# IvanBanny/para-ortho-pca-bo

Measured on AMD Instinct MI355X. Metric: BO iterations/sec (incl. GP refit + EI opt), BBOB f15 d=40, higher is better.
Workload: dtype f64; 1 GPU; configs[1]: PCA_BO on BBOB f15 d=40, budget=450, n_DoE=120, EI, var_threshold=0.95; one run per GPU (run list f15/d40/instances 0..N-1 partitioned by pcabo.sharding), timed steps spread evenly over the 330 BO iterations of the run; num_restarts=10, raw_samples=512, batch_limit=5, maxiter=200, parallelism=run-parallel x1

## Files before the change

include/pcabo.h:

```cpp
#ifndef PCABO_H
#define PCABO_H

#include <stddef.h>
#include <stdint.h>

#ifdef __cplusplus
extern "C" {
#endif

typedef struct pcabo_ctx pcabo_ctx;

typedef enum {
  PCABO_OK = 0,
  PCABO_ERR_ARG = -1,
  PCABO_ERR_NOT_PD = -2,
  PCABO_ERR_HIP = -3,
  PCABO_ERR_NAN = -4,
  PCABO_ERR_TIMEOUT = -5
} pcabo_status;

enum { PCABO_KERNEL_MATERN52 = 0, PCABO_KERNEL_RBF = 1 };
enum { PCABO_ACQ_LOG_EI = 0, PCABO_ACQ_PI = 1, PCABO_ACQ_UCB = 2 };
enum { PCABO_PTR_HOST = 0, PCABO_PTR_DEVICE = 1 };

int pcabo_abi_version(void);

int pcabo_device_count(void);

int pcabo_ctx_create(int device, int max_n, int max_d, int max_q, pcabo_ctx** out);
int pcabo_ctx_destroy(pcabo_ctx* ctx);
int pcabo_set_pointer_mode(pcabo_ctx* ctx, int mode);
int pcabo_last_error(pcabo_ctx* ctx, char* buf, int buflen);

enum { PCABO_OPT_RESIDENT = 0, PCABO_OPT_BESTF_F32 = 1, PCABO_OPT_GROUP_ACQ = 2,
       PCABO_OPT_DEVICE_LBFGSB = 3 ,
       PCABO_OPT_HIDDEN_TAIL = 5  };
int pcabo_set_option(pcabo_ctx* ctx, int option, int value);

int pcabo_wpca(pcabo_ctx* ctx, const double* X, const double* f, const int64_t* ranks, int n, int d,
               int maximize, double var_threshold, int n_components, const double* noise,
               double* data_mean, double* pca_mean, double* comps, double* evr, int* k, double* Z);

int pcabo_gp_condition(pcabo_ctx* ctx, const double* Z, const double* y, int n, int k,
                       const double* norm_bounds, double lengthscale, double noise, int kernel);

int pcabo_gp_condition_begin(pcabo_ctx* ctx, const double* Z, const double* y, int n, int k,
                             const double* norm_bounds, double lengthscale, double noise, int kernel);
int pcabo_gp_condition_end(pcabo_ctx* ctx);

int pcabo_gp_condition_end_eval(pcabo_ctx* ctx, const double* Xq, int q, double best_f, int maximize, int acq,
                                double* val);

int pcabo_gp_mll(pcabo_ctx* ctx, const double* Z , const double* y, int n, int k,
                 const double* norm_bounds, int kernel, const double* theta , double* loss, double* grad );
#define PCABO_FIT_TASK_NOT_PD (-2)
#define PCABO_FIT_TASK_DOMAIN (-3)
int pcabo_gp_fit(pcabo_ctx* ctx, const double* Z, const double* y, int n, int k, const double* norm_bounds, int kernel,
                 double* theta_inout , double* loss, int* info );
int pcabo_gp_mll_ard(pcabo_ctx* ctx, const double* Z, const double* y, int n, int k, const double* norm_bounds, int kernel,
                     const double* theta , double* loss, double* grad );
int pcabo_gp_fit_ard(pcabo_ctx* ctx, const double* Z, const double* y, int n, int k, const double* norm_bounds, int kernel,
                     double* theta_inout , double* loss, int* info );

int pcabo_wpca_gp_condition_begin(pcabo_ctx* ctx, const double* X, const double* f, const int64_t* ranks, int n,
                                  int d, int maximize, double var_threshold, int n_components, const double* noise,
                                  const double* y, double lengthscale, double gp_noise, int kernel,
                                  double* data_mean, double* pca_mean, double* comps, double* evr, int* k);

int pcabo_wpca_results(pcabo_ctx* ctx, double* data_mean, double* pca_mean, double* comps, double* evr, int* k);

int pcabo_acq_bounds(pcabo_ctx* ctx, double* bounds);

int pcabo_acq_eval(pcabo_ctx* ctx, const double* Xq, int q, double best_f, int maximize, int acq,
                   double* val, double* grad);
int pcabo_logei(pcabo_ctx* ctx, const double* Xq, int q, double best_f, int maximize,
                double* val, double* grad);

enum { PCABO_POST_OBS_NOISE = 1 };
int pcabo_gp_posterior(pcabo_ctx* ctx, const double* Xq, int q, int flags, double* mean, double* var, double* cov);

enum { PCABO_POST_CENTRED = 2 };
#define PCABO_POST_MAX_SAMPLES 1024
int pcabo_gp_posterior_sample(pcabo_ctx* ctx, const double* Xq, int q, int flags, const double* base, int S,
                              double* samples, double* mean , double* jitter_used );

int pcabo_gp_loo(pcabo_ctx* ctx, double* mean , double* var , double* z , double* lpd , double* lpd_sum );

enum { PCABO_EXTEND_BELIEVER = 1 };
int pcabo_gp_extend(pcabo_ctx* ctx, const double* Zp, const double* yp, int p, int flags);
int pcabo_gp_truncate(pcabo_ctx* ctx, int n0);
int pcabo_gp_extended(pcabo_ctx* ctx, int* n_base , int* n );

int pcabo_optimize_acqf(pcabo_ctx* ctx, const double* ics, int num_restarts, int batch_limit,
                        const double* bounds, int maxiter, double best_f, int maximize, int acq,
                        double* cand, double* vals, int* info, int* failed);

int pcabo_inverse_map(pcabo_ctx* ctx, const double* z, double* x);

int pcabo_get_gp_state(pcabo_ctx* ctx, double* K_chol , double* Rinv ,
                       double* alpha , double* y_mean_std , double* norm_bounds );
int pcabo_get_gram(pcabo_ctx* ctx, double* K );

typedef double (*pcabo_fg_callback)(const double* x, double* g, void* user);
int pcabo_lbfgsb_minimize(int nvar, double* x, const double* lower, const double* upper,
                          pcabo_fg_callback fg, void* user, int m, double factr, double pgtol,
                          int maxiter, int maxfun, int maxls, double* f_out, int* nit, int* nfev,
                          int* task_out);
int pcabo_lbfgsb_set_vector_kernels(int enabled);
int pcabo_lbfgsb_set_sum_order(int order);

int pcabo_sobol_scramble(int64_t* state, const int64_t* ltm, int k);
int pcabo_sobol_draw(const int64_t* state, const int64_t* shift, int k, int n, const double* lo, const double* rng, double* out);
int pcabo_sobol_draw_rows(const int64_t* const* states, const int64_t* const* shifts, const int* ks, int rows, int n,
                          const double* boxes, long long box_stride, double* const* outs);
int pcabo_torch_randint2(void* blob, int64_t count, int64_t* out);
int pcabo_torch_multinomial_rows(void* const* blobs, const double* weights, int rows, int n, int n_pick, int64_t* out);
int pcabo_boltzmann_pick_rows(void* const* blobs, const double* vals, int rows, int n, int n_pick, double eta, int64_t* out, int* flags);

int pcabo_set_profiling(pcabo_ctx* ctx, int enabled);
int pcabo_get_profile_calibration(pcabo_ctx* ctx, double* pair_ms, double* empty_kernel_ms);
int pcabo_get_profile(pcabo_ctx* ctx, int which, double* ms, int64_t* launches, double* bytes, double* flops);
int pcabo_reset_profile(pcabo_ctx* ctx);

typedef struct pcabo_batch pcabo_batch;
int pcabo_batch_create(int device, int B, int max_n, int max_d, int max_q, pcabo_batch** out);
int pcabo_batch_destroy(pcabo_batch* batch);
int pcabo_batch_set_workers(pcabo_batch* batch, int workers);
int pcabo_batch_set_option(pcabo_batch* batch, int option, int value);
int pcabo_device_lbfgsb_limits(int* max_n, int* max_k, int* max_group);
int pcabo_batch_last_error(pcabo_batch* batch, char* buf, int buflen);
pcabo_ctx* pcabo_batch_ctx(pcabo_batch* batch, int b);

int pcabo_batch_set_input_strides(pcabo_batch* batch, size_t x_stride, size_t noise_stride, size_t y_stride);
int pcabo_batch_wpca_gp_condition_begin(pcabo_batch* batch, const double* X, const int64_t* ranks, const double* noise,
                                        const double* y, int n, int d, int maximize, double var_threshold,
                                        int n_components, double lengthscale, double gp_noise, int kernel);
int pcabo_batch_gp_condition_begin(pcabo_batch* batch, const double* Z, const double* y, int n, int k, const double* norm_bounds,
                                   double lengthscale, double gp_noise, int kernel);
int pcabo_batch_wpca_results(pcabo_batch* batch, double* data_mean, double* pca_mean, double* comps, double* evr, int* k);
int pcabo_batch_acq_bounds(pcabo_batch* batch, double* bounds);
int pcabo_batch_gp_condition_end_eval(pcabo_batch* batch, const double* Xq, int q, const double* best_f, int maximize,
                                      int acq, double* val, int* status);
int pcabo_batch_acq_score(pcabo_batch* batch, const double* Xq , int q, const double* best_f , int maximize,
                          int acq, double* val , int* status );
int pcabo_batch_acq_score_begin(pcabo_batch* batch, const double* Xq, int q, const double* best_f, int maximize, int acq);
int pcabo_batch_acq_score_end(pcabo_batch* batch, int q, double* val, int* status);
int pcabo_batch_gp_posterior(pcabo_batch* batch, const double* Xq, int q, int flags, double* mean, double* var, double* cov,
                             int* status);
int pcabo_batch_gp_posterior_sample(pcabo_batch* batch, const double* Xq , int q, int flags,
                                    const double* base , int S, double* samples ,
                                    double* mean , double* jitter_used , int* status );
int pcabo_batch_gp_loo(pcabo_batch* batch, double* mean , double* var, double* z, double* lpd, double* lpd_sum ,
                       int* status );
int pcabo_batch_gp_extend(pcabo_batch* batch, const double* Zp , const double* yp , int p, int flags,
                          int* status );
int pcabo_batch_gp_truncate(pcabo_batch* batch, int n0, int* status );
int pcabo_batch_gp_extended(pcabo_batch* batch, int* n_base, int* n);
int pcabo_batch_optimize_acqf(pcabo_batch* batch, const double* ics, int num_restarts, int batch_limit,
                              const double* bounds, int maxiter, const double* best_f, int maximize, int acq,
                              double* cand, double* vals, int* info, int* failed, int* status);
int pcabo_batch_busy(pcabo_batch* batch);
int pcabo_batch_gp_condition_end_eval_begin(pcabo_batch* batch, const double* Xq, int q, const double* best_f, int maximize, int acq);
int pcabo_batch_gp_condition_end_eval_end(pcabo_batch* batch, const double* Xq, int q, const double* best_f, int maximize,
                                          int acq, double* val, int* status);
int pcabo_batch_optimize_acqf_begin(pcabo_batch* batch, const double* ics, int num_restarts, int batch_limit,
                                    const double* bounds, int maxiter, const double* best_f, int maximize, int acq);
int pcabo_batch_optimize_acqf_end(pcabo_batch* batch, int num_restarts, int batch_limit, double* cand, double* vals, int* info,
                                  int* failed, int* status);
int pcabo_batch_inverse_map_begin(pcabo_batch* batch, const double* z);
int pcabo_batch_inverse_map_end(pcabo_batch* batch, double* x);
int pcabo_batch_set_active(pcabo_batch* batch, const int* active);
int pcabo_batch_set_profiling(pcabo_batch* batch, int enabled);
int pcabo_batch_get_profile(pcabo_batch* batch, double* ms);
int pcabo_batch_inverse_map(pcabo_batch* batch, const double* z, double* x);
int pcabo_batch_device_acq_eval(pcabo_batch* batch, const double* Xq, int q, const double* best_f, int maximize, int acq,
                                double* val, double* grad);
int pcabo_batch_gp_mll(pcabo_batch* batch, const double* theta , double* loss , double* grad , int* status );
int pcabo_batch_gp_fit(pcabo_batch* batch, double* theta_inout , double* loss , int* info , int* status );
// ... 25 lines not shown
```

para-ortho-pca-bo_amd/Algorithms/BayesianOptimization/DeviceBayesianOptimizer.py:

```python
from __future__ import annotations

import os
import warnings
from abc import abstractmethod
from contextlib import contextmanager
from typing import Callable, Optional, Union

import numpy as np

from pcabo import _native
from pcabo import acqopt as _acqopt
from pcabo.acqopt import ALLOWED_ACQUISITION_FUNCTION_STRINGS, ALLOWED_SHORTHAND_ACQUISITION_FUNCTION_STRINGS
from pcabo.gcguard import RunGuard
from .AbstractBayesianOptimizer import AbstractBayesianOptimizer

LENGTHSCALE = 0.6931471805599453
NOISE = 0.006737946999085467


def checked_ard(ard, fit_gp) -> bool:
    if ard and not fit_gp:
        raise ValueError("ard=True fits one lengthscale per input: it needs fit_gp=True")
    return bool(ard)


def fit_gp_hyperparameters(ctx, y, Z=None, norm_bounds=None, ard=False) -> dict:
    if ard:
        hp = ctx.gp_fit_ard(y, Z=Z, norm_bounds=norm_bounds)
    else:
        hp = ctx.gp_fit(y, Z=Z, norm_bounds=norm_bounds, kernel=_native.KERNEL_MATERN52)
    if hp["warnflag"] != 0:
        warnings.warn(f"GP hyperparameter fit did not converge (warnflag {hp['warnflag']}, task {hp['task']}); keeping the last "
                      "accepted iterate", RuntimeWarning)
    return hp


class AnalyticAcquisitionFunction:
    acq_code = _native.ACQ_LOG_EI

    def __init__(self, model=None, best_f: float = 0.0, maximize: bool = True):
        self.model, self.best_f, self.maximize = model, best_f, maximize

    @property
    def device_scalar(self) -> float:
        return self.best_f


class LogExpectedImprovement(AnalyticAcquisitionFunction):
    acq_code = _native.ACQ_LOG_EI


class ProbabilityOfImprovement(AnalyticAcquisitionFunction):
    acq_code = _native.ACQ_PI


class UpperConfidenceBound(AnalyticAcquisitionFunction):
    acq_code = _native.ACQ_UCB

    def __init__(self, model=None, beta=None, maximize: bool = True, **kwargs):
        if kwargs or beta is None:
            raise TypeError("UpperConfidenceBound.__init__() got an unexpected keyword argument 'best_f'")
        super().__init__(model, 0.0, maximize)
        self.beta = beta
        self.kappa = _acqopt.ucb_kappa(beta)

    @property
    def device_scalar(self) -> float:
        return self.kappa


_ACQUISITION_CLASSES = dict(zip(ALLOWED_ACQUISITION_FUNCTION_STRINGS,
                                (LogExpectedImprovement, ProbabilityOfImprovement, UpperConfidenceBound)))


class DeviceBayesianOptimizer(AbstractBayesianOptimizer):
    ODD_NAME = "Oddly defined name"
    FINAL_LINE = "Optimization Process finalized!"

    def __init__(self, budget: int, n_DoE: int = 0, acquisition_function: str = "expected_improvement",
                 random_seed: int = 43, **kwargs):
        self._device = int(kwargs.pop("device", 0))
        self._record_trace = bool(kwargs.pop("record_trace", False))
        self._guard = RunGuard(kwargs.pop("torch_threads", 4), kwargs.pop("gc_freeze", True))
        self._resident = bool(kwargs.pop("resident", True))
        self._fantasy_points = int(kwargs.pop("fantasy_points", 0))
        if self._fantasy_points < 0:
            raise ValueError("fantasy_points must be >= 0")
        self._fit_gp = bool(kwargs.pop("fit_gp", False))
        self._ard = checked_ard(kwargs.pop("ard", False), self._fit_gp)
        self.gp_hyperparameters = None
        self._ucb_beta = _acqopt.checked_ucb_beta(kwargs.pop("ucb_beta", None), acquisition_function)
        self._q, self._q_strategy = _acqopt.checked_q(kwargs.pop("q", 1), kwargs.pop("q_strategy", "kriging_believer"))
        super().__init__(budget, n_DoE, **kwargs)
        self.random_seed = random_seed
        smoke_test = os.environ.get("SMOKE_TEST")
        self._torch_config = {
            "device": f"hip:{self._device}",
            "dtype": np.float64,
            "SMOKE_TEST": smoke_test,
            "BATCH_SIZE": 3 if not smoke_test else 2,
            "NUM_RESTARTS": 10 if not smoke_test else 2,
            "RAW_SAMPLES": 512 if not smoke_test else 32,
        }
        self._acq_func_class = None
        self._acq_func = None
        self.acquisition_function_name = acquisition_function
        self._ctx: Optional[_native.Context] = None
        self.lbfgsb_info = []
        self.trace = []
        self.phase_breakdown = {}

    def __call__(self, problem: Union[Callable, object], dim: Optional[int] = -1,
                 bounds: Optional[np.ndarray] = None, **kwargs) -> None:
        try:
            self._start(problem, dim, bounds, **kwargs)
            for _ in range(self.budget - self.n_DoE):
                if self.number_of_function_evaluations >= self.budget:
                    break
                self._bo_iteration(problem, **kwargs)
        finally:
            self._finish()

    def _start(self, problem, dim=-1, bounds=None, **kwargs) -> None:
        self._guard.enter()
        self.impose_random_seed()
        AbstractBayesianOptimizer.__call__(self, problem, dim, bounds, **kwargs)
        if self._pbar is not None:
            self._pbar.update(self.n_DoE)
        self._ctx = _native.Context(max_n=self.budget + self._fantasy_points, max_d=self.dimension,
                                    max_q=max(self._torch_config["RAW_SAMPLES"], 16), device=self._device)
        if not self._resident:
            self._ctx.set_option(_native.OPT_RESIDENT, 0)
        self._open_run(problem)

    def _bo_iteration(self, problem, **kwargs) -> None:
        if self._record_trace:
            import torch
            self.trace.append({"n": len(self.f_evals), "numpy_state": np.random.get_state(),
                               "torch_state": torch.get_rng_state(), "best_f": self.current_best})
        self._condition_model(**kwargs)
        self._ctx.match_best_f_dtype(self.current_best)
        if self._ucb_beta is not None:
            self.acquisition_function = self.acquisition_function_class(
                model=self._ctx, beta=self._ucb_beta, maximize=self.maximization)
        else:
            self.acquisition_function = self.acquisition_function_class(
                model=self._ctx, best_f=self.current_best, maximize=self.maximization)
        for candidate in self.optimize_acqf_and_get_observation():
            if self.number_of_function_evaluations >= self.budget:
                break
            new_f = self._observe(problem, candidate)
            if self._pbar is not None:
                self._pbar.update(1)
            self.f_evals.append(new_f)
            self.number_of_function_evaluations += 1
        self.assign_new_best()
        if self.verbose:
            print(f"Evaluations: {self.number_of_function_evaluations}/{self.budget}",
                  f"Best: x:{self.x_evals[self.current_best_index]} y:{self.current_best}", flush=True)

    def _finish(self) -> None:
        self._close_run()
        self._guard.leave()
        if self._ctx is not None:
            self._ctx.close()
            self._ctx = None
        if self.verbose:
            print(self.FINAL_LINE)
        self.restore_random_states()

    def _q_eff(self) -> int:
        return max(1, min(self._q, self.budget - len(self.f_evals)))

    def assign_new_best(self):
        super().assign_new_best()

    @abstractmethod
    def _condition_model(self, **kwargs) -> None:
        """From the evaluated points to this iteration's GP in the context."""

    @abstractmethod
    def optimize_acqf_and_get_observation(self) -> np.ndarray:
        """The iteration's candidates (`_q_eff()` of them), one row each, in the space of the model."""

    @abstractmethod
    def _observe(self, problem, candidate) -> float:
        """Append the candidate's point to x_evals and return its objective value."""

    def _open_run(self, problem) -> None:
        """Set-up of the subclass, the context is open."""

    def _close_run(self) -> None:
        """Tear-down of the subclass, in front of the shared one; also called after a start that failed."""

    def _model_ready(self) -> bool:
        return True

    def _to_model_space(self, X: np.ndarray) -> np.ndarray:
        return X

    def _model_input(self, query: str, X=None):
        if self._ctx is None or not self._model_ready():
            raise RuntimeError(f"{query}: no run is open, or the model of the current iteration is not conditioned yet")
        if X is not None:
            return self._to_model_space(np.asarray(X, dtype=np.float64).reshape(-1, self.dimension))

    def posterior(self, X, observation_noise: bool = False, covariance: bool = False) -> dict:
        Z = self._model_input("posterior", X)
        return self._ctx.gp_posterior(Z, observation_noise, covariance)

    def posterior_samples(self, X, n_samples=1, seed=None, base_samples=None, observation_noise: bool = False,
                          centred: bool = False) -> dict:
        Z = self._model_input("posterior_samples", X)
        return self._ctx.gp_posterior_samples(Z, None if base_samples is not None else n_samples, base_samples, seed,
                                              observation_noise, centred)

    def loo(self) -> dict:
        self._model_input("loo")
        return self._ctx.gp_loo()

    @contextmanager
    def fantasy(self, X, y=None):
        Z = self._model_input("fantasy", X)
        n0 = self._ctx.n
        self._ctx.gp_extend(Z, y)
        try:
            yield self
        finally:
            self._ctx.gp_truncate(n0)

    @property
    def device_context(self):
        return self._ctx

    @property
    def torch_config(self) -> dict:
        return self._torch_config

    @property
    def acquisition_function_name(self) -> str:
        return self._acquisition_function_name

    @acquisition_function_name.setter
    def acquisition_function_name(self, new_name: str) -> None:
        self._acquisition_function_name = _acqopt.acquisition_long_name(new_name, self.ODD_NAME)
        self.set_acquisition_function_subclass()

    def set_acquisition_function_subclass(self) -> None:
        if self._acquisition_function_name in _ACQUISITION_CLASSES:
            self._acq_func_class = _ACQUISITION_CLASSES[self._acquisition_function_name]

    @property
    def acquisition_function_class(self) -> Callable:
# ... 14 lines not shown
```

para-ortho-pca-bo_amd/Algorithms/BayesianOptimization/PCA_BO.py:

```python
from __future__ import annotations

import warnings
from time import perf_counter

import numpy as np

from pcabo import _native
from pcabo import initializers as _init
from pcabo import acqopt as _acqopt
from .DeviceBayesianOptimizer import (
    ALLOWED_ACQUISITION_FUNCTION_STRINGS, ALLOWED_SHORTHAND_ACQUISITION_FUNCTION_STRINGS, AnalyticAcquisitionFunction,
    DeviceBayesianOptimizer, LogExpectedImprovement, ProbabilityOfImprovement, UpperConfidenceBound, LENGTHSCALE, NOISE,
    checked_ard, fit_gp_hyperparameters)

OOB_PENALTY = 1000


class _FittedPCA:

    def __init__(self, components, mean, evr, k):
        self.components_ = components[:k]
        self.mean_ = mean
        self.explained_variance_ratio_ = evr
        self.n_components_ = components.shape[0]
# ... 134 lines not shown
                                                   daemon=True)
            self.__noise_thread.start()
        self.__noise_pending = True
        self.__noise_req.put((n + q_eff, self.dimension))

    def _stop_noise_worker(self) -> None:
        if self.__noise_thread is None:
            return
        self.__noise_req.put(None)
        self.__noise_thread.join()
        self.__noise_thread, self.__noise_pending = None, False
        self.__noise_req = self.__noise_res = None

    def _transform_points_to_reduced_space(self) -> None:
        if len(self.x_evals) < 2:
            if len(self.x_evals) == 1:
                self.__z_evals = [np.zeros(1)]
            return
        X = self._design_matrix()
        ranks = self._calculate_ranks()
        noise = self._take_noise(X.shape)
        start = perf_counter()
        if self.__fused and not self._fit_gp:
            self._ctx.wpca_gp_condition(
                X, np.array(self.f_evals, dtype=np.float64), ranks=ranks, maximize=self.maximization,
                var_threshold=self.var_threshold, n_components=self.n_components, noise=noise,
                lengthscale=LENGTHSCALE, gp_noise=NOISE, kernel=_native.KERNEL_MATERN52, collect=False)
            self.__gp_pending = True
            self.__engine_ready, guess, saved = None, None, None
            k_prev = self.reduced_space_dim_num
            if self.__speculate_engine and k_prev:
                import torch
                saved = torch.get_rng_state()
                guess = _init.scrambled_sobol_engine(int(k_prev))
            res = self._ctx.wpca_results()
            if guess is not None:
                if res["k"] == k_prev:
                    self.__engine_ready = guess
                else:
                    torch.set_rng_state(saved)
        else:
            res = self._ctx.wpca(X, ranks=ranks, maximize=self.maximization, var_threshold=self.var_threshold,
                                  n_components=self.n_components, noise=noise, want_Z=False, want_full=True)
        self.timing_logs["pca"].append(perf_counter() - start)
        self.data_mean = res["data_mean"]
        self.component_matrix = res["components"]
        self.explained_variance_ratio = res["evr"]
        self.reduced_space_dim_num = res["k"]
        self.pca = _FittedPCA(res["components"], res["pca_mean"], res["evr"], res["k"])
        if self.verbose:
            k = res["k"]
            print(f"Using {k} principal components with {np.sum(res['evr'][:k]) * 100:.2f}% explained variance")
        self.__z_evals = [res["k"]] * X.shape[0]

    def _initialize_model(self, **kwargs):
        if not self.__z_evals:
            return
        start = perf_counter()
        if self.__gp_pending:
            self.timing_logs["SingleTaskGP"].append(perf_counter() - start)
            return
        if self._fit_gp:
            self.gp_hyperparameters = fit_gp_hyperparameters(self._ctx, np.array(self.f_evals, dtype=np.float64), ard=self._ard)
            self.timing_logs["SingleTaskGP"].append(perf_counter() - start)
            return
        self._ctx.gp_condition(np.array(self.f_evals, dtype=np.float64), lengthscale=LENGTHSCALE, noise=NOISE,
                                kernel=_native.KERNEL_MATERN52, wait=False)
        self.__gp_pending = True
        self.timing_logs["SingleTaskGP"].append(perf_counter() - start)

    def optimize_acqf_and_get_observation(self) -> np.ndarray:
        ctx, cfg = self._ctx, self._torch_config
        acq = self.acquisition_function
        num_restarts, raw_samples, batch_limit = cfg["NUM_RESTARTS"], cfg["RAW_SAMPLES"], 5
        start = perf_counter()
        engine, self.__engine_ready = self.__engine_ready, None
        if engine is None:
            engine = _init.scrambled_sobol_engine(ctx.k)
        bounds = ctx.acq_bounds()
        t0 = perf_counter()
        raw = _init.draw_sobol(bounds, raw_samples, engine)
        self.phase_breakdown["sobol"] = self.phase_breakdown.get("sobol", 0.0) + perf_counter() - t0
        raw_vals = None
        if self.__gp_pending and self.__early_scoring:
            t0 = perf_counter()
            raw_vals = ctx.gp_wait_eval(raw, acq.device_scalar, acq.maximize, acq.acq_code)
            self.__gp_pending = False
            self.phase_breakdown["raw_eval"] = self.phase_breakdown.get("raw_eval", 0.0) + perf_counter() - t0
        elif self.__gp_pending:
            ctx.gp_wait()
            self.__gp_pending = False
        new_z, infos = _acqopt.propose(
            ctx, bounds, acq.device_scalar, acq.maximize, acq.acq_code, num_restarts, raw_samples, batch_limit, 200,
            q_eff=self._q_eff(), strategy=self._q_strategy, f_evals=self.f_evals,
            raw=raw, raw_vals=raw_vals, breakdown=self.phase_breakdown,
            trace=self.trace[-1] if self._record_trace else None,
            before_lbfgsb=self._prefetch_noise)
        self.timing_logs["optimize_acqf"].append(perf_counter() - start)
        self.lbfgsb_info.extend(infos)
        return new_z

    def _transform_point_to_original_space(self, z: np.ndarray) -> np.ndarray:
        if self.pca is None:
            return np.random.uniform(self.bounds[:, 0], self.bounds[:, 1])
        return self._ctx.inverse_map(z)

    def reset(self):
        super().reset()
        self.__z_evals = []
        self.pca = None
        self.explained_variance_ratio = None
```

para-ortho-pca-bo_amd/Algorithms/BayesianOptimization/Vanilla_BO.py:

```python
from __future__ import annotations

from time import perf_counter

import numpy as np

from pcabo import _native
from pcabo import acqopt as _acqopt
from pcabo import initializers as _init
from .DeviceBayesianOptimizer import DeviceBayesianOptimizer, LENGTHSCALE, NOISE, fit_gp_hyperparameters


class Vanilla_BO(DeviceBayesianOptimizer):
    TIME_PROFILES = ["SingleTaskGP", "optimize_acqf"]
    ODD_NAME = "Oddly defined name {name}"
    FINAL_LINE = "Optimisation Process finalized!"

    def __str__(self):
        return "This is an instance of a Vanilla BO Optimizer"

    def _open_run(self, problem) -> None:
        d = self.dimension
        self.__identity = np.vstack([np.zeros(d), np.ones(d)])
        self.__box = np.ascontiguousarray(self.bounds.T, dtype=np.float64)

    def _condition_model(self, **kwargs) -> None:
        self._initialise_model(**kwargs)

    def _observe(self, problem, candidate) -> float:
        x = np.asarray(candidate, dtype=np.float64).ravel()
        self.x_evals.append(x)
        return problem(x)

    def _initialise_model(self, **kwargs):
        X = np.array(self.x_evals, dtype=np.float64).reshape((-1, self.dimension))
        y = np.array(self.f_evals, dtype=np.float64)
        start = perf_counter()
        if self._fit_gp:
            self.gp_hyperparameters = fit_gp_hyperparameters(self._ctx, y, Z=X, norm_bounds=self.__identity, ard=self._ard)
            self.timing_logs["SingleTaskGP"].append(perf_counter() - start)
            return
        self._ctx.gp_condition(y, Z=X, norm_bounds=self.__identity, lengthscale=LENGTHSCALE, noise=NOISE,
                               kernel=_native.KERNEL_MATERN52, wait=False)
        self.timing_logs["SingleTaskGP"].append(perf_counter() - start)

    def optimize_acqf_and_get_observation(self) -> np.ndarray:
        ctx, cfg, acq = self._ctx, self._torch_config, self.acquisition_function
        start = perf_counter()
        engine = _init.scrambled_sobol_engine(self.dimension)
        raw = _init.draw_sobol(self.__box, cfg["RAW_SAMPLES"], engine)
        raw_vals = None
        if not self._fit_gp:
            t0 = perf_counter()
            raw_vals = ctx.gp_wait_eval(raw, acq.device_scalar, acq.maximize, acq.acq_code)
            self.phase_breakdown["raw_eval"] = self.phase_breakdown.get("raw_eval", 0.0) + perf_counter() - t0
        new_x, infos = _acqopt.propose(
            ctx, self.__box, acq.device_scalar, acq.maximize, acq.acq_code, cfg["NUM_RESTARTS"], cfg["RAW_SAMPLES"], 5, 200,
            q_eff=self._q_eff(), strategy=self._q_strategy, f_evals=self.f_evals, raw=raw, raw_vals=raw_vals, breakdown=self.phase_breakdown,
            trace=self.trace[-1] if self._record_trace else None)
        self.timing_logs["optimize_acqf"].append(perf_counter() - start)
        self.lbfgsb_info.extend(infos)
        return new_x
```

para-ortho-pca-bo_amd/csrc/host_entry.cpp:

```cpp
#include "../../include/pcabo.h"
#include "lbfgsb.h"

#include <algorithm>
#include <atomic>
#include <cmath>
#include <cstdint>
#include <cstring>
#include <vector>

extern "C" {

namespace {
std::atomic<int> g_minimize_sum_order{0};
thread_local unsigned g_last_branches[LBB_COUNT] = {};
}

int pcabo_lbfgsb_minimize(int nvar, double* x, const double* lower, const double* upper, pcabo_fg_callback fg,
                          void* user, int m, double factr, double pgtol, int maxiter, int maxfun, int maxls,
                          double* f_out, int* nit, int* nfev, int* task_out) {
  if (nvar < 1 || !x || !fg || m < 1) return PCABO_ERR_ARG;
  LbfgsbDriver run;
  run.init(nvar, x, lower, upper, g_minimize_sum_order.load(), maxiter, maxfun, m, factr, pgtol, maxls);
  while (run.advance()) run.absorb(fg(run.x.data(), run.g.data(), user));
  std::copy(run.x.begin(), run.x.end(), x);
  if (f_out) *f_out = run.f;
  if (nit) *nit = run.niter;
  if (nfev) *nfev = run.nfev;
  if (task_out) *task_out = run.opt.task();
  { std::vector<double> end((size_t)nvar); run.end_point(end.data()); }
  std::copy(run.opt.branches(), run.opt.branches() + LBB_COUNT, g_last_branches);
  return run.opt.warnflag();
}

int pcabo_debug_lbfgsb_branch_names(char* buf, int cap) {
  if (buf && cap > 0) {
    size_t at = 0;
    buf[0] = 0;
    for (int i = 0; i < LBB_COUNT; ++i) {
      const char* nm = lbfgsb_branch_name(i);
      const size_t len = strlen(nm);
      if (at + len + 2 > (size_t)cap) break;
      if (i) buf[at++] = ',';
      memcpy(buf + at, nm, len + 1);
      at += len;
    }
  }
  return LBB_COUNT;
}
int pcabo_debug_lbfgsb_branches(unsigned* out, int cap) {
  if (out) for (int i = 0; i < LBB_COUNT && i < cap; ++i) out[i] = g_last_branches[i];
  return LBB_COUNT;
}

int pcabo_lbfgsb_set_vector_kernels(int enabled) { return lbfgsb_set_vector_kernels(enabled); }
int pcabo_lbfgsb_set_sum_order(int order) { return g_minimize_sum_order.exchange(order ? 1 : 0); }

int pcabo_sobol_scramble(int64_t* state, const int64_t* ltm, int k) {
  if (!state || !ltm || k < 1) return PCABO_ERR_ARG;
  const int MAXBIT = 30;
  for (int d = 0; d < k; ++d) {
    int64_t col[30];
    for (int c = 0; c < MAXBIT; ++c) col[c] = (int64_t)1 << (MAXBIT - 1 - c);
    for (int p = 1; p < MAXBIT; ++p) {
      const int64_t* row = ltm + ((size_t)d * MAXBIT + p) * MAXBIT;
      const int64_t pbit = (int64_t)1 << (MAXBIT - 1 - p);
      for (int c = 0; c < p; ++c) col[c] |= (row[c] & 1) ? pbit : 0;
    }
    for (int j = 0; j < MAXBIT; ++j) {
      unsigned long long v = (unsigned long long)state[(size_t)d * MAXBIT + j] & ((1ull << MAXBIT) - 1);
      int64_t t2 = 0;
      while (v) {
        const int b = __builtin_ctzll(v);
        t2 ^= col[MAXBIT - 1 - b];
        v &= v - 1;
      }
      state[(size_t)d * MAXBIT + j] = t2;
    }
  }
  return PCABO_OK;
}

int pcabo_sobol_draw(const int64_t* state, const int64_t* shift, int k, int n, const double* lo, const double* rng, double* out) {
  if (!state || !shift || !out || k < 1 || n < 1 || (lo == nullptr) != (rng == nullptr)) return PCABO_ERR_ARG;
  const int MAXBIT = 30;
  const double recip = 9.31322574615478515625e-10;
  std::vector<int64_t> q(shift, shift + k);
  for (int i = 0; i < n; ++i) {
    if (i > 0) {
      unsigned v = (unsigned)(i - 1);
      int l = 0;
      while (v & 1u) { v >>= 1; ++l; }
      if (l >= MAXBIT) return PCABO_ERR_ARG;
      for (int j = 0; j < k; ++j) q[j] ^= state[(size_t)j * MAXBIT + l];
    }
    double* o = out + (size_t)i * k;
    for (int j = 0; j < k; ++j) {
      const double u = i == 0 ? (double)((float)q[j]) * recip : (double)q[j] * recip;
      if (lo) { const double t = rng[j] * u; o[j] = lo[j] + t; }
      else o[j] = u;
    }
  }
  return PCABO_OK;
}


int pcabo_sobol_draw_rows(const int64_t* const* states, const int64_t* const* shifts, const int* ks, int rows, int n,
                          const double* boxes, long long box_stride, double* const* outs) {
  if (!states || !shifts || !ks || !boxes || !outs || rows < 1 || n < 1 || n > (1 << 30)) return PCABO_ERR_ARG;
  for (int r = 0; r < rows; ++r)
    if (states[r] && (ks[r] < 1 || !shifts[r] || !outs[r])) return PCABO_ERR_ARG;
  std::vector<double> rng;
  for (int r = 0; r < rows; ++r) {
    if (!states[r]) continue;
    const int k = ks[r];
    const double* lo = boxes + (size_t)r * box_stride;
    rng.resize(k);
    for (int j = 0; j < k; ++j) rng[j] = lo[k + j] - lo[j];
    pcabo_sobol_draw(states[r], shifts[r], k, n, lo, rng.data(), outs[r]);
  }
  return PCABO_OK;
}

namespace {
struct TorchMt {
  uint64_t seed; int32_t left; int32_t seeded; uint64_t next; uint64_t state[624];
};
inline uint32_t mt_twist(uint64_t u, uint64_t v) {
  return (uint32_t)((((uint32_t)u & 0x80000000u) | ((uint32_t)v & 0x7fffffffu)) >> 1) ^ (((uint32_t)v & 1u) ? 0x9908b0dfu : 0u);
}
__attribute__((optimize("O3"))) inline void mt_next_state(TorchMt* s) {
  constexpr int N = 624, M = 397;
  uint64_t* __restrict__ st = s->state;
  for (int i = 0; i < N - M; ++i) st[i] = (uint32_t)st[i + M] ^ mt_twist(st[i], st[i + 1]);
  for (int i = N - M; i < N - 1; ++i) st[i] = (uint32_t)st[i + M - N] ^ mt_twist(st[i], st[i + 1]);
  st[N - 1] = (uint32_t)st[M - 1] ^ mt_twist(st[N - 1], st[0]);
  s->left = N;
  s->next = 0;
}
inline uint32_t mt_draw(TorchMt* s) {
  if (--s->left == 0) mt_next_state(s);
  uint32_t y = (uint32_t)s->state[s->next++];
  y ^= (y >> 11);
  y ^= (y << 7) & 0x9d2c5680u;
  y ^= (y << 15) & 0xefc60000u;
  y ^= (y >> 18);
  return y;
}
__attribute__((optimize("O3"))) inline void mt_temper_bits(const uint64_t* w, int64_t m, int64_t* out) {
  for (int64_t i = 0; i < m; ++i) {
    uint32_t y = (uint32_t)w[i];
    y ^= (y >> 11);
    y ^= (y << 7) & 0x9d2c5680u;
    y ^= (y << 15) & 0xefc60000u;
    y ^= (y >> 18);
    out[i] = (int64_t)(y & 1u);
  }
}
}

int pcabo_torch_randint2(void* blob, int64_t count, int64_t* out) {
  if (!blob || !out || count < 0) return PCABO_ERR_ARG;
  TorchMt* s = static_cast<TorchMt*>(blob);
  if (!s->seeded || s->left < 1 || s->left > 624 || s->next > 624) return PCABO_ERR_ARG;
  while (count > 0) {
    int64_t take;
    if (s->left == 1) {
      mt_next_state(s);
      take = count < 624 ? count : 624;
      mt_temper_bits(s->state + s->next, take, out);
      s->next += (uint64_t)take;
      s->left = 624 - (int32_t)(take - 1);
    } else {
      take = count < s->left - 1 ? count : s->left - 1;
      mt_temper_bits(s->state + s->next, take, out);
      s->next += (uint64_t)take;
      s->left -= (int32_t)take;
    }
    out += take;
    count -= take;
  }
  return PCABO_OK;
}

namespace {
void multinomial_row(TorchMt* s, const double* w, int n, int n_pick, double* ratio, int* best, int64_t* out) {
  for (int i = 0; i < n; ++i) {
    const uint64_t hi = mt_draw(s), lo = mt_draw(s);
    const uint64_t r64 = (hi << 32) | lo;
    const double u = (double)(r64 & ((1ull << 53) - 1)) * 1.1102230246251565e-16;
    const double q = -std::log1p(-u);
    ratio[i] = w[i] / q;
  }
  int have = 0;
  for (int i = 0; i < n; ++i) {
    const double v = ratio[i];
    if (have == n_pick && !(v > ratio[best[have - 1]])) continue;
    int pos = have < n_pick ? have : n_pick - 1;
    while (pos > 0 && v > ratio[best[pos - 1]]) { if (pos < n_pick) best[pos] = best[pos - 1]; --pos; }
    best[pos] = i;
    if (have < n_pick) ++have;
  }
  for (int j = 0; j < n_pick; ++j) out[j] = best[j];
}
}

namespace {
void boltzmann_rows(void* const* blobs, const double* vals, int r0, int r1, int n, int n_pick, double eta, int64_t* out, int* flags) {
  std::vector<double> w((size_t)n), ratio((size_t)n);
  std::vector<int> best((size_t)n_pick);
  for (int r = r0; r < r1; ++r) {
    TorchMt* s = static_cast<TorchMt*>(blobs[r]);
    if (!s) { flags[r] = 2; continue; }
    const double* v = vals + (size_t)r * n;
    double mean = 0.0, m2 = 0.0;
    int arg = 0;
    for (int i = 0; i < n; ++i) {
      const double d = v[i] - mean;
      mean += d / (double)(i + 1);
      m2 += d * (v[i] - mean);
      if (v[i] > v[arg]) arg = i;
    }
    const double sd = std::sqrt(m2 / (double)(n - 1));
    if (!(sd > 0.0)) { flags[r] = 1; continue; }
    double scale = eta;
    for (;;) {
      bool inf = false;
      for (int i = 0; i < n; ++i) { w[i] = std::exp(scale * ((v[i] - mean) / sd)); inf = inf || std::isinf(w[i]); }
      if (!inf) break;
      scale *= 0.5;
    }
    int64_t* o = out + (size_t)r * n_pick;
    multinomial_row(s, w.data(), n, n_pick, ratio.data(), best.data(), o);
    bool has = false;
    for (int j = 0; j < n_pick; ++j) has = has || o[j] == arg;
    if (!has) o[n_pick - 1] = arg;
    flags[r] = 0;
  }
}
}

int pcabo_boltzmann_pick_rows(void* const* blobs, const double* vals, int rows, int n, int n_pick, double eta, int64_t* out, int* flags) {
  if (!blobs || !vals || !out || !flags || rows < 1 || n < 2 || n_pick < 1 || n_pick > n) return PCABO_ERR_ARG;
  for (int r = 0; r < rows; ++r) {
    const TorchMt* s = static_cast<const TorchMt*>(blobs[r]);
    if (s && (!s->seeded || s->left < 1 || s->left > 624 || s->next > 624)) return PCABO_ERR_ARG;
  }
  boltzmann_rows(blobs, vals, 0, rows, n, n_pick, eta, out, flags);
  return PCABO_OK;
}

int pcabo_torch_multinomial_rows(void* const* blobs, const double* weights, int rows, int n, int n_pick, int64_t* out) {
  if (!blobs || !weights || !out || rows < 1 || n < 1 || n_pick < 1 || n_pick > n) return PCABO_ERR_ARG;
  std::vector<double> ratio((size_t)n);
  std::vector<int> best((size_t)n_pick);
  for (int r = 0; r < rows; ++r) {
    TorchMt* s = static_cast<TorchMt*>(blobs[r]);
    if (!s) continue;
    if (!s->seeded || s->left < 1 || s->left > 624 || s->next > 624) return PCABO_ERR_ARG;
    multinomial_row(s, weights + (size_t)r * n, n, n_pick, ratio.data(), best.data(), out + (size_t)r * n_pick);
  }
  return PCABO_OK;
}

}
```

para-ortho-pca-bo_amd/csrc/host_selftest.cpp:

```cpp
#include "../../include/pcabo.h"
#include "host_side.h"
#include "lb_plan.h"
#include "ctx_layout.h"
#include "model_state.h"

#include <atomic>
#include <cmath>
#include <cstdint>
#include <cstdio>
#include <cstdlib>
#include <cstring>
#include <vector>

namespace {

int g_fail = 0;
#define CHECK(c, ...) do { if (!(c)) { std::fprintf(stderr, "FAIL %s:%d: ", __FILE__, __LINE__); std::fprintf(stderr, __VA_ARGS__); std::fprintf(stderr, "\n"); ++g_fail; } } while (0)

struct Lcg {
  uint64_t s;
  explicit Lcg(uint64_t seed) : s(seed * 6364136223846793005ull + 1442695040888963407ull) {}
  double uni() { s = s * 6364136223846793005ull + 1442695040888963407ull; return (double)(s >> 11) * (1.0 / 9007199254740992.0); }
};

// ... 22 lines not shown
      for (int i = 0; i < nvar; ++i) { o.c[i] = 4.0 * r.uni() - 2.0; lo[i] = -1.0 - r.uni(); hi[i] = 1.0 + r.uni(); x[i] = 6.0 * r.uni() - 3.0; }
      double f = 0.0; int nit = 0, nfev = 0, task = 0;
      const int wf = pcabo_lbfgsb_minimize(nvar, x.data(), lo.data(), hi.data(), fg_objective, &o, 10, 1e7, 1e-5, 200, 15000, 20, &f, &nit, &nfev, &task);
      CHECK(wf >= 0 && wf <= 2, "warnflag %d", wf);
      CHECK(std::isfinite(f) && nfev >= 1, "f %g nfev %d", f, nfev);
      for (int i = 0; i < nvar; ++i) CHECK(x[i] >= lo[i] && x[i] <= hi[i], "x[%d] = %g outside the box", i, x[i]);
    }
  }
  pcabo_lbfgsb_set_vector_kernels(1);
  pcabo_lbfgsb_set_sum_order(0);
  {
    const int nvar = 12;
    Objective o; o.c.assign(nvar, 0.5);
    std::vector<double> x(nvar, 2.0), lo(nvar, -INFINITY), hi(nvar, INFINITY);
    for (int i = 0; i < nvar; i += 3) lo[i] = 0.75;
    for (int i = 1; i < nvar; i += 3) hi[i] = 0.25;
    double f = 0.0; int nit = 0, nfev = 0, task = 0;
    const int wf = pcabo_lbfgsb_minimize(nvar, x.data(), lo.data(), hi.data(), fg_objective, &o, 17, 1e7, 1e-5, 200, 15000, 20, &f, &nit, &nfev, &task);
    CHECK(wf == 0, "half-bounded problem: warnflag %d task %d", wf, task);
  }
  CHECK(pcabo_lbfgsb_minimize(0, nullptr, nullptr, nullptr, fg_objective, nullptr, 10, 1e7, 1e-5, 1, 1, 20, nullptr, nullptr, nullptr, nullptr) == PCABO_ERR_ARG, "bad arguments accepted");
}

void test_sobol() {
  for (int k : {1, 3, 36, 89}) {
    Lcg r(5 + k);
    std::vector<int64_t> state((size_t)k * 30), ltm((size_t)k * 30 * 30), shift(k);
    for (auto& v : state) v = (int64_t)(r.uni() * 1073741824.0);
    for (auto& v : ltm) v = r.uni() < 0.5 ? 0 : 1;
    for (auto& v : shift) v = (int64_t)(r.uni() * 1073741824.0);
    CHECK(pcabo_sobol_scramble(state.data(), ltm.data(), k) == PCABO_OK, "scramble");
    for (int n : {1, 2, 512, 513}) {
      std::vector<double> lo(k, -1.5), rng(k, 3.0), out((size_t)n * k, -7.0);
      CHECK(pcabo_sobol_draw(state.data(), shift.data(), k, n, lo.data(), rng.data(), out.data()) == PCABO_OK, "draw");
      for (double v : out) CHECK(v >= -1.5 && v <= 1.5, "sample %g outside the box", v);
      CHECK(pcabo_sobol_draw(state.data(), shift.data(), k, n, nullptr, nullptr, out.data()) == PCABO_OK, "draw (unit cube)");
      for (double v : out) CHECK(v >= 0.0 && v < 1.0, "unit sample %g", v);
    }
  }
}

void test_torch_rng() {
  struct Blob { uint64_t seed; int32_t left, seeded; uint64_t next; uint64_t state[624]; unsigned char tail[32]; };
  const int rows = 70, n = 512, n_pick = 10;
  std::vector<Blob> blobs(rows), again;
  std::vector<double> vals((size_t)rows * n);
  for (int r = 0; r < rows; ++r) {
    Lcg g(900 + r);
    blobs[r].seed = 900 + r; blobs[r].left = 1 + (r * 37) % 624; blobs[r].seeded = 1; blobs[r].next = 624 - blobs[r].left;
    for (auto& w : blobs[r].state) w = (uint64_t)(g.uni() * 4294967296.0);
    for (auto& c : blobs[r].tail) c = 0;
    for (int i = 0; i < n; ++i) vals[(size_t)r * n + i] = r == 5 ? 1.25 : 40.0 * g.uni() - 20.0;
  }
  again = blobs;
  std::vector<void*> ptr(rows);
  for (int r = 0; r < rows; ++r) ptr[r] = &blobs[r];
  ptr[7] = nullptr;
  std::vector<int64_t> out((size_t)rows * n_pick, -1), out1((size_t)rows * n_pick, -1);
  std::vector<int> flags(rows, -1), flags1(rows, -1);
  CHECK(pcabo_boltzmann_pick_rows(ptr.data(), vals.data(), rows, n, n_pick, 1.0, out.data(), flags.data()) == PCABO_OK, "pick rows");
  for (int r = 0; r < rows; ++r) {
    void* p1 = r == 7 ? nullptr : (void*)&again[r];
    CHECK(pcabo_boltzmann_pick_rows(&p1, vals.data() + (size_t)r * n, 1, n, n_pick, 1.0, out1.data() + (size_t)r * n_pick, flags1.data() + r) == PCABO_OK, "pick row %d", r);
    CHECK(flags[r] == flags1[r] && flags[r] == (r == 7 ? 2 : r == 5 ? 1 : 0), "flag of row %d: %d / %d", r, flags[r], flags1[r]);
    if (flags[r] != 0) continue;
    for (int j = 0; j < n_pick; ++j) {
      CHECK(out[(size_t)r * n_pick + j] == out1[(size_t)r * n_pick + j], "row %d pick %d differs between the all-rows call and the one-row call", r, j);
      CHECK(out[(size_t)r * n_pick + j] >= 0 && out[(size_t)r * n_pick + j] < n, "row %d pick %d out of range", r, j);
    }
    CHECK(blobs[r].left == again[r].left && blobs[r].next == again[r].next && blobs[r].state[0] == again[r].state[0], "generator of row %d", r);
  }
  std::vector<int64_t> bits(2000);
  CHECK(pcabo_torch_randint2(&blobs[0], 2000, bits.data()) == PCABO_OK, "randint2");
  for (int64_t b : bits) CHECK(b == 0 || b == 1, "bit %lld", (long long)b);
  std::vector<double> w((size_t)3 * n);
  Lcg g(77);
  for (auto& v : w) v = 0.01 + g.uni();
  void* three[3] = {&blobs[1], nullptr, &blobs[2]};
  std::vector<int64_t> idx(3 * n_pick, -1);
  CHECK(pcabo_torch_multinomial_rows(three, w.data(), 3, n, n_pick, idx.data()) == PCABO_OK, "multinomial rows");
  for (int j = 0; j < n_pick; ++j) CHECK(idx[j] >= 0 && idx[j] < n && idx[n_pick + j] == -1 && idx[2 * n_pick + j] >= 0, "multinomial pick %d", j);
  blobs[3].left = 900;
  CHECK(pcabo_torch_randint2(&blobs[3], 4, bits.data()) == PCABO_ERR_ARG, "a broken blob accepted");
}

void test_sobol_rows() {
  const int rows = 37, n = 130, kmax = 36;
  int ks[rows];
  for (int r = 0; r < rows; ++r) ks[r] = r == 0 ? 3 : r == 2 ? 1 : 1 + (r * 7) % 36;
  std::vector<std::vector<int64_t>> st(rows), sh(rows);
  std::vector<double> boxes((size_t)rows * 2 * kmax, NAN), out((size_t)rows * n * kmax, -7.0), one((size_t)n * kmax);
  std::vector<const int64_t*> sp(rows), hp(rows);
  std::vector<double*> op(rows);
  for (int r = 0; r < rows; ++r) {
    Lcg g(40 + r);
    st[r].resize((size_t)ks[r] * 30); sh[r].resize(ks[r]);
    for (auto& v : st[r]) v = (int64_t)(g.uni() * 1073741824.0);
    for (auto& v : sh[r]) v = (int64_t)(g.uni() * 1073741824.0);
    for (int j = 0; j < ks[r]; ++j) { boxes[(size_t)r * 2 * kmax + j] = -1.0 - j; boxes[(size_t)r * 2 * kmax + ks[r] + j] = 2.0 + r; }
    sp[r] = r == 2 ? nullptr : st[r].data(); hp[r] = sh[r].data(); op[r] = out.data() + (size_t)r * n * kmax;
  }
  CHECK(pcabo_sobol_draw_rows(sp.data(), hp.data(), ks, rows, n, boxes.data(), 2 * kmax, op.data()) == PCABO_OK, "draw rows");
  for (int r = 0; r < rows; ++r) {
    if (r == 2) { CHECK(op[r][0] == -7.0, "a skipped run was written"); continue; }
    std::vector<double> rng(ks[r]);
    for (int j = 0; j < ks[r]; ++j) rng[j] = boxes[(size_t)r * 2 * kmax + ks[r] + j] - boxes[(size_t)r * 2 * kmax + j];
    CHECK(pcabo_sobol_draw(st[r].data(), sh[r].data(), ks[r], n, boxes.data() + (size_t)r * 2 * kmax, rng.data(), one.data()) == PCABO_OK, "draw");
    for (int i = 0; i < n * ks[r]; ++i) CHECK(one[i] == op[r][i], "run %d element %d", r, i);
    if (ks[r] < kmax) CHECK(op[r][(size_t)n * ks[r]] == -7.0, "write behind the points of run %d", r);
  }
}

void test_plan() {
  std::vector<int> plan(LB_PLAN_INTS + 64, 0x5a5a5a5a);
  for (int NP = 64; NP <= LB_MAXNP; NP += 64) {
    const int S = NP / 64;
    for (int n = NP - 63; n <= NP; ++n) {
      lb_build_plan_t(plan.data(), n, S);
      for (int i = LB_PLAN_INTS; i < (int)plan.size(); ++i) CHECK(plan[i] == 0x5a5a5a5a, "write behind the plan (n %d)", n);
      for (int pass = 0; pass < 2; ++pass) {
        const int* pw = plan.data() + pass * LB_PLAN_PASS;
        std::vector<int> cover(S * 512, 0);
        int max_dest = -1;
        for (int w = 0; w < LB_WAVES; ++w) {
          const int* e = pw + w * LB_PLAN_WAVE;
          CHECK(e[0] >= 0 && e[0] <= 2, "segments of a wave: %d", e[0]);
          for (int g = 0; g < e[0]; ++g) {
            const int u = e[1 + 4 * g], a = e[2 + 4 * g], b = e[3 + 4 * g], dest = e[4 + 4 * g];
            CHECK(u >= 0 && u < S && a >= 0 && b <= NP && a < b, "segment (%d, %d, %d)", u, a, b);
            CHECK(dest >= -1 && dest < lb_max_slots(NP), "slot %d of %d (n %d NP %d)", dest, lb_max_slots(NP), n, NP);
            if (dest > max_dest) max_dest = dest;
            for (int t = a; t < b && u >= 0 && u < S && t >= 0 && t < 512; ++t) cover[u * 512 + t] += 1;
          }
        }
        for (int u = 0; u < S; ++u) {
          const int lo = pass == 0 ? 0 : 64 * u, hi = pass == 0 ? (n < 64 * (u + 1) ? n : 64 * (u + 1)) : (n > 64 * u ? n : 64 * u);
          for (int t = 0; t < 512; ++t) CHECK(cover[u * 512 + t] == ((t >= lo && t < hi) ? 1 : 0), "pass %d unit %d index %d covered %d times (n %d)", pass, u, t, cover[u * 512 + t], n);
        }
      }
    }
  }
}

void drive_group(RestartGroup& rg, Objective& o, std::vector<double>* trail) {
  std::vector<double> hVal(rg.q0 + rg.nq), hGrad((size_t)(rg.q0 + rg.nq) * rg.k);
  while (rg.advance()) {
    if (trail) trail->insert(trail->end(), rg.x.begin(), rg.x.end());
    for (int j = 0; j < rg.nq; ++j) {
      double* gj = hGrad.data() + (size_t)(rg.q0 + j) * rg.k;
      hVal[rg.q0 + j] = -fg_objective(rg.x.data() + (size_t)j * rg.k, gj, &o);
      for (int c = 0; c < rg.k; ++c) gj[c] = -gj[c];
    }
    CHECK(rg.absorb(hVal.data(), hGrad.data(), rg.q0), "NaN gradient");
  }
}

struct Joint { Objective* o; int nq, k; };
double fg_joint(const double* x, double* g, void* user) {
  const Joint* J = static_cast<const Joint*>(user);
  double f = 0.0;
  for (int j = 0; j < J->nq; ++j) f += fg_objective(x + (size_t)j * J->k, g + (size_t)j * J->k, J->o);
  return f;
}

void test_restart_group() {
  const int k = 9, nq = 4, q0 = 3, restarts = q0 + nq;
// ... 872 lines not shown
    expect_state(r[0], {3, 3, 2, 1, 4, 64, LS, S2, KN, 0.0, T, F, 0, 0, F, F, F, F, 4, F, 1, 2}, "member 0 behind the wPCA results");
    expect_state(r[2], {3, 3, 2, 5, 8, 64, LS, S2, KN, 0.0, T, F, 0, 0, F, F, F, F, 4, F, 1, 2}, "member 2 behind the wPCA results");
    expect_answers(r[0], {F, GP_NONE, T, T, F, F, T}, "member 0 behind the wPCA results");
    expect_answers(r[2], {F, GP_NONE, T, F, F, F, T}, "member 2 behind the wPCA results");
    b.scoring_begun();
    expect_batch({3, 3, 2, 0, 0, 64, LS, S2, KN, 0.0, T, F, 3, 2, T, F, F, F, 4, F, 1, 2}, F, T, F, F, GP_IN_FLIGHT, T, T, "scoring enqueued");
    b.scoring_ended();
    r[1].condition_failed(); r[2].condition_ended_ok(1e-7);
    const bool ok[3] = {T, F, T};
    for (int i = 0; i < 3; ++i) r[i].follow(b, r[i].own().ended(ok[i]));
    expect_batch({3, 3, 2, 0, 0, 64, LS, S2, KN, 0.0, T, F, 3, 2, F, T, F, F, 4, F, 1, 2}, F, F, F, F, GP_READY, F, T, "scoring collected");
    expect_state(r[0], {3, 3, 2, 1, 4, 64, LS, S2, KN, 0.0, T, F, 0, 0, F, T, F, F, 4, F, 1, 2}, "member 0 conditioned");
    expect_state(r[1], {3, 3, 2, 5, 8, 64, LS, S2, KN, 0.0, T, F, 0, 0, F, F, F, F, 4, F, 1, 2}, "member 1 without a GP");
    expect_state(r[2], {3, 3, 2, 5, 8, 64, LS, S2, KN, 1e-7, T, F, 0, 0, F, T, F, F, 4, F, 1, 2}, "member 2 on rung 1e-7");
    expect_answers(r[0], {F, GP_READY, T, T, F, F, T}, "member 0 conditioned");
    expect_answers(r[1], {F, GP_NONE, T, F, F, F, T}, "member 1 without a GP");
    expect_answers(r[2], {F, GP_READY, T, F, F, F, T}, "member 2 on rung 1e-7");
    b.opt_begun(8, 4);
    CHECK(b.opt_matches(8, 4) && !b.opt_matches(8, 5) && !b.opt_matches(7, 4) && b.gp_ready() == GP_IN_FLIGHT && b.begin_pending(), "optimisation enqueued");
    b.opt_ended();
    CHECK(!b.opt_matches(8, 4) && b.gp_ready() == GP_READY, "optimisation collected");
    b.imap_begun(); CHECK(b.imap_enqueued && b.gp_ready() == GP_IN_FLIGHT, "inverse map enqueued");
    b.imap_ended(); CHECK(!b.begin_pending() && b.gp_ready() == GP_READY, "inverse map collected");
    b.m.wpca_enqueued(64, 2);
    CHECK(!b.tickets_reset_if_needed(slabs(64), runs), "same slab count, nobody dirty: no reset");
    b.condition_enqueued(64, 2, -1, LS, S2, KN);
    for (int i = 0; i < 3; ++i) r[i].follow(b, r[i].own().with_k(r[i].k).started(LS, S2));
    b.wpca_collected();
    for (int i = 0; i < 3; ++i) r[i].follow(b, r[i].own().with_k(ks[i]));
    expect_state(r[2], {64, 64, 2, 5, 8, 64, LS, S2, KN, 0.0, T, F, 0, 0, F, F, F, F, 4, F, 0, 2}, "member 2 behind the second conditioning");
    expect_answers(r[2], {F, GP_NONE, T, F, T, F, T}, "member 2 behind the second conditioning");
    const double ls_own[3] = {0.5, LS, 1.0}, s2_own[3] = {0.01, S2, 0.02};
    for (int i = 0; i < 3; ++i) r[i].follow(b, r[i].own().started(ls_own[i], s2_own[i]));
    expect_state(r[0], {64, 64, 2, 1, 4, 64, 0.5, 0.01, KN, 0.0, T, F, 0, 0, F, F, F, F, 4, F, 0, 2}, "member 0 in a fit round");
    expect_answers(r[0], {F, GP_NONE, T, F, F, F, T}, "member 0 in a fit round");
    r[2].condition_ended_ok(1e-8);
    r[0].follow(b, r[0].own().ended(true)); r[1].follow(b, r[1].own().ended(true));
    b.fit_finished();
    r[1].follow(b, r[1].own().ended(false));
    expect_batch({64, 64, 2, 0, 0, 64, LS, S2, KN, 0.0, T, F, 64, 2, F, T, F, F, 4, F, 0, 2}, T, F, F, F, GP_READY, T, T, "fit finished");
    expect_state(r[0], {64, 64, 2, 1, 4, 64, 0.5, 0.01, KN, 0.0, T, F, 0, 0, F, T, F, F, 4, F, 0, 2}, "member 0 fitted");
    expect_state(r[1], {64, 64, 2, 5, 8, 64, LS, S2, KN, 0.0, T, F, 0, 0, F, F, F, F, 4, F, 0, 2}, "member 1 after a failed fit");
    expect_state(r[2], {64, 64, 2, 5, 8, 64, 1.0, 0.02, KN, 1e-8, T, F, 0, 0, F, T, F, F, 4, F, 0, 2}, "member 2 fitted on rung 1e-8");
    expect_answers(r[0], {F, GP_READY, T, F, F, F, T}, "member 0 fitted");
    expect_answers(r[1], {F, GP_NONE, T, F, T, F, T}, "member 1 after a failed fit");
    expect_answers(r[2], {F, GP_READY, T, F, T, F, T}, "member 2 fitted on rung 1e-8");
    for (int i = 0; i < 3; ++i) r[i].follow(b, r[i].own().with_k(ks[i]));
    expect_state(r[0], {64, 64, 2, 1, 4, 64, 0.5, 0.01, KN, 0.0, T, F, 0, 0, F, T, F, F, 4, F, 0, 2}, "member 0 keeps its fitted model");
    expect_answers(r[0], {F, GP_READY, T, F, F, F, T}, "member 0 keeps its fitted model");
    CHECK(b.tickets_reset_if_needed(slabs(128), runs), "65 points: reset");
    b.condition_enqueued(65, 5, 5, LS, S2, KN);
    for (int i = 0; i < 3; ++i) { r[i].rt_rebuilt(); r[i].follow(b, r[i].own().with_k(5).started(LS, S2)); }
    expect_batch({65, 65, 5, 5, 8, 128, LS, S2, KN, 0.0, F, F, 64, 2, T, F, F, F, 8, F, 0, 2}, F, F, F, F, GP_IN_FLIGHT, T, T, "conditioning without a wPCA");
    expect_state(r[0], {65, 65, 5, 5, 8, 128, LS, S2, KN, 0.0, F, F, 0, 0, F, F, F, F, 8, F, 0, 2}, "member 0 behind it");
    expect_answers(r[0], {F, GP_NONE, F, F, F, T, F}, "member 0 behind the conditioning without a wPCA");
    {
      BatchState c2 = b; c2.m.wpca_enqueued(65, 5); c2.condition_enqueued(65, 5, -1, LS, S2, KN);
      CHECK(c2.m.wpca_uncollected && !c2.wpca_on_host(), "k on the device: the wPCA is uncollected");
      c2.condition_enqueued(65, 5, 5, LS, S2, KN);
      CHECK(!c2.m.wpca_uncollected && c2.wpca_on_host(), "k known: no wPCA goes with the conditioning");
    }
    r[1].launch_may_have_died();
    CHECK(b.tickets_need_reset(8, runs) && !b.m.tickets_need_reset(8), "a member's mark makes the batch's reset due at an unchanged NP");
    r[1].follow(b, r[1].own().ended(true));
    CHECK(r[1].cnt_dirty && b.tickets_need_reset(8, runs), "following the batch does not clear a member's mark");
    CHECK(b.tickets_reset_if_needed(8, runs), "the next conditioning resets");
    CHECK(!b.m.cnt_dirty && !r[0].cnt_dirty && !r[1].cnt_dirty && !r[2].cnt_dirty && r[1].cnt_S == 8, "the reset clears the mark on the batch and on every member");
    CHECK(!b.tickets_need_reset(8, runs) && b.tickets_need_reset(4, runs), "no mark, same slab count: no reset");
    r[0].condition_ended_ok(0.0);
    r[0].gram_fetched(); CHECK(r[0].rt_stale, "Gram fetched: stale");
    r[0].rt_rebuilt(); CHECK(!r[0].rt_stale, "the conditioning's rebuild: fresh");
    r[0].n_changed(66); CHECK(r[0].rt_stale && r[0].n_base == 65, "extend: stale, n_base held");
  }
}

}

int main(int argc, char** argv) {
  const int workers = argc > 1 ? std::atoi(argv[1]) : 4;
  test_minimize();
  test_sobol();
  test_sobol_rows();
  test_torch_rng();
  test_plan();
  test_restart_group();
  test_crew();
  test_free_pair();
  test_fit_run();
  test_inverse_map_host();
  test_ctx_layout();
  test_model_state();
  test_gang_pool(1, 3);
  test_gang_pool(workers, 11);
  if (g_fail) { std::fprintf(stderr, "host selftest: %d check(s) failed\n", g_fail); return 1; }
  std::printf("host selftest ok\n");
  return 0;
}
```

para-ortho-pca-bo_amd/csrc/host_side.h:

```cpp
#pragma once
#include "../../include/pcabo.h"
#include "lbfgsb.h"

#include <algorithm>
#include <atomic>
#include <cassert>
#include <chrono>
#include <cmath>
#include <condition_variable>
#include <cstring>
#include <functional>
#include <memory>
#include <mutex>
#include <thread>
#include <utility>
#include <vector>

struct RestartGroup : LbfgsbDriver {
  int q0 = 0, nq = 0, k = 0;
  std::vector<double> lo, hi, vc;
  void init(const double* ics, const double* bounds, int q0_, int nq_, int k_, int maxiter, int sum_order = 0) {
    q0 = q0_; nq = nq_; k = k_;
    lo.resize(nq * k); hi.resize(nq * k);
    for (int j = 0; j < nq; ++j)
      for (int c = 0; c < k; ++c) { lo[j * k + c] = bounds[c]; hi[j * k + c] = bounds[k + c]; }
    LbfgsbDriver::init(nq * k, ics + (size_t)q0 * k, lo.data(), hi.data(), sum_order, maxiter);
  }
  bool absorb(const double* hVal, const double* hGrad, int row) {
    double fs = 0.0;
    bool nan = false;
    for (int j = 0; j < nq; ++j) fs += hVal[row + j];
    for (int t = 0; t < nq * k; ++t) {
      const double gv = -hGrad[(size_t)row * k + t];
      if (gv != gv) nan = true;
      g[t] = gv;
    }
    if (nan) return false;
    LbfgsbDriver::absorb(-fs);
    vc.assign(hVal + row, hVal + row + nq);
    return true;
  }
};

struct RunRestarts {
  std::vector<RestartGroup> grp;
  int status = PCABO_OK;
  double* xq = nullptr;
  const double *val = nullptr, *grad = nullptr;
  void init(const double* ics, const double* bounds, int num_restarts, int batch_limit, int k, int maxiter, int sum_order = 0) {
    grp.resize((num_restarts + batch_limit - 1) / batch_limit);
    for (size_t gi = 0; gi < grp.size(); ++gi) {
      const int q0 = (int)gi * batch_limit;
      grp[gi].init(ics, bounds, q0, std::min(batch_limit, num_restarts - q0), k, maxiter, sum_order);
    }
    status = PCABO_OK;
  }
  void bind(double* xq_, const double* val_, const double* grad_) { xq = xq_; val = val_; grad = grad_; }
  template <class Redo> int end_points(double* cand, double* vals, Redo&& redo) {
    int n = 0;
    for (RestartGroup& rg : grp) {
      if (rg.end_point(cand + (size_t)rg.q0 * rg.k)) std::copy(rg.vc.begin(), rg.vc.end(), vals + rg.q0);
      else { redo(rg); ++n; }
    }
    return n;
  }
  int end_points(double* cand, double* vals) { return end_points(cand, vals, [](const RestartGroup&) {}); }
  bool report(int* info, size_t slot0) const {
    bool any = false;
    for (size_t gi = 0; gi < grp.size(); ++gi) {
      const RestartGroup& rg = grp[gi];
      const int wf = rg.opt.warnflag();
      if (info) { int* o = info + 4 * (slot0 + gi); o[0] = rg.niter; o[1] = rg.nfev; o[2] = wf; o[3] = rg.opt.task(); }
      if (wf == 2) any = true;
    }
    return any;
  }
};

inline unsigned group_entry(int run, int q0, int nq) { return ((unsigned)run << 16) | ((unsigned)q0 << 8) | (unsigned)nq; }
inline unsigned query_entry(int run, int q) { return ((unsigned)run << 16) | (unsigned)q; }

template <class Stage, class Eval>
int run_rounds(RunRestarts* runs, const std::vector<int>& order, Stage&& stage, Eval&& eval) {
  std::vector<std::pair<RunRestarts*, RestartGroup*>> pend;
  size_t ng = 0;
  for (int b : order) ng += runs[b].grp.size();
  pend.reserve(ng);
  for (;;) {
    pend.clear();
    for (int b : order) {
      RunRestarts& run = runs[b];
      if (run.status != PCABO_OK) continue;
      for (RestartGroup& rg : run.grp) {
        if (!rg.advance()) continue;
        std::memcpy(run.xq + (size_t)rg.q0 * rg.k, rg.x.data(), rg.x.size() * sizeof(double));
        stage(b, rg);
        pend.push_back({&run, &rg});
      }
    }
    if (pend.empty()) return PCABO_OK;
    const int rc = eval();
    if (rc != PCABO_OK) return rc;
    for (auto& pe : pend)
      if (!pe.second->absorb(pe.first->val, pe.first->grad, pe.second->q0)) pe.first->status = PCABO_ERR_NAN;
  }
}

struct OptHelper {
  std::thread th;
  std::mutex mu;
  std::condition_variable cv;
  std::atomic<unsigned> go{0}, done{0};
  std::atomic<bool> quit{false}, active{false};
  std::function<void()> fn;
  void run() {
    unsigned seen = 0;
    while (true) {
      {
        std::unique_lock<std::mutex> lk(mu);
        cv.wait(lk, [&] { return active.load(std::memory_order_acquire) || quit.load(std::memory_order_acquire); });
      }
      if (quit.load(std::memory_order_acquire)) return;
      while (active.load(std::memory_order_acquire)) {
        const unsigned cur = go.load(std::memory_order_acquire);
        if (cur == seen) { __builtin_ia32_pause(); continue; }
        seen = cur;
        fn();
        done.store(cur, std::memory_order_release);
      }
    }
  }
  void start() { if (!th.joinable()) th = std::thread([this] { run(); }); }
  void begin(std::function<void()> f) {
    start();
    fn = std::move(f);
    { std::lock_guard<std::mutex> lk(mu); active.store(true, std::memory_order_release); }
    cv.notify_one();
  }
  void end() { active.store(false, std::memory_order_release); }
  void shutdown() {
    if (!th.joinable()) return;
    { std::lock_guard<std::mutex> lk(mu); quit.store(true, std::memory_order_release); active.store(false, std::memory_order_release); }
    cv.notify_one();
    th.join();
  }
  unsigned post() {
    const unsigned ticket = go.load(std::memory_order_relaxed) + 1;
    go.store(ticket, std::memory_order_release);
    return ticket;
  }
  void wait(unsigned ticket) const { while (done.load(std::memory_order_acquire) != ticket) __builtin_ia32_pause(); }
};

struct OptCrew {
  OptHelper helper;
  std::vector<std::unique_ptr<OptHelper>> more;
  void shutdown() {
    helper.shutdown();
    for (auto& h : more) h->shutdown();
    more.clear();
  }
};

inline int stepping_threads(int ngroups) { return ngroups >= 12 ? std::min(7, 1 + ngroups / 8) : 2; }
struct CrewCall {
  std::vector<RestartGroup>& grp;
  std::vector<char>& pending;
  const int ngroups, T;
  OptHelper* hs[6];
  int nh = 0;
  CrewCall(OptCrew& crew, RunRestarts& run, std::vector<char>& pending_)
      : grp(run.grp), pending(pending_), ngroups((int)run.grp.size()), T(stepping_threads((int)run.grp.size())) {
    if (T > 2) while ((int)crew.more.size() < T - 2) crew.more.emplace_back(new OptHelper());
    if (ngroups > 1) hs[nh++] = &crew.helper;
    for (int i = 0; i < T - 2; ++i) hs[nh++] = crew.more[i].get();
    for (int i = 0; i < nh; ++i) hs[i]->begin(share(i + 1));
  }
  CrewCall(const CrewCall&) = delete;
  ~CrewCall() { for (int i = 0; i < nh; ++i) hs[i]->end(); }
  void advance(int gi) {
    if (pending[gi]) pending[gi] = 0;
    else grp[gi].advance();
  }
  void step_share(int first) { for (int gi = first; gi < ngroups; gi += T) advance(gi); }
  std::function<void()> share(int first) { return [this, first] { step_share(first); }; }
  void advance_all() {
    unsigned tickets[6];
    for (int i = 0; i < nh; ++i) tickets[i] = hs[i]->post();
    step_share(0);
    for (int i = 0; i < nh; ++i) hs[i]->wait(tickets[i]);
  }
  template <class F1, class F0> void beside(F1&& f1, F0&& f0) {
    OptHelper& hp = *hs[0];
    hp.fn = std::forward<F1>(f1);
    const unsigned ticket = hp.post();
    f0();
    hp.wait(ticket);
    hp.fn = share(1);
  }
};

inline int pack_active(RunRestarts& run, std::vector<int>& qoff) {
  int nq = 0;
  for (size_t gi = 0; gi < run.grp.size(); ++gi) {
    const RestartGroup& rg = run.grp[gi];
    qoff[gi] = -1;
    if (!rg.active) continue;
    qoff[gi] = nq;
    std::memcpy(run.xq + (size_t)nq * rg.k, rg.x.data(), rg.x.size() * sizeof(double));
    nq += rg.nq;
  }
  return nq;
}
inline bool absorb_packed(RunRestarts& run, const std::vector<int>& qoff) {
  for (size_t gi = 0; gi < run.grp.size(); ++gi)
    if (qoff[gi] >= 0 && !run.grp[gi].absorb(run.val, run.grad, qoff[gi])) return false;
  return true;
}

struct FreePair {
  bool timed_out[2] = {false, false}, got_nan[2] = {false, false};
  bool slow_first[2] = {false, false};
  unsigned long long used[2] = {0, 0};
};
template <class Mailbox>
void free_group(RestartGroup& rg, int gi, Mailbox& mb, const double* val, const double* grad, unsigned long long seq0,
                std::atomic<int>& abort_flag, char& pending, FreePair& out, std::chrono::nanoseconds timeout,
                std::chrono::nanoseconds slow) {
  const int q0 = rg.q0, nq = rg.nq;
  unsigned long long r = 0;
  for (;;) {
    if (abort_flag.load(std::memory_order_relaxed)) { pending = 1; break; }
    const unsigned long long tag = seq0 + (++r);
    mb.post(q0, nq, rg.x.data(), tag);
    const auto t0 = std::chrono::steady_clock::now();
    unsigned long spins = 0;
    bool ok = true;
    for (int j = 0; j < nq && ok; ++j) {
      while (mb.tag_of(q0 + j) != tag) {
// ... 226 lines not shown
```

para-ortho-pca-bo_amd/csrc/pcabo_api.hip:

```cpp
#include "../../include/pcabo.h"
#include "pcabo_internal.h"
#include "lbfgsb.h"
#include "host_side.h"
#include "model_state.h"

#include <algorithm>
#include <atomic>
#include <chrono>
#include <thread>
#include <condition_variable>
#include <functional>
#include <mutex>
#include <cstdlib>
#include <cmath>
#include <cstdio>
#include <cstring>
#include <new>
#include <optional>
#include <vector>
#include <dirent.h>
#include <fcntl.h>
#include <signal.h>
#include <stdint.h>
#include <cerrno>
#include <unistd.h>
#include <emmintrin.h>

#define PCABO_ABI_VERSION 2
#define PROF_GROUPS 6
#define PROF_POOL 4096

struct ProfPair { hipEvent_t a, b; int group; double bytes, flops; };

struct pcabo_ctx {
  int device = 0;
  hipStream_t stream = nullptr;
  hipEvent_t evBounds = nullptr;
  hipEvent_t evPca = nullptr;
  hipStream_t stream2 = nullptr;
  hipEvent_t evZn = nullptr, evKS = nullptr;
  bool opt_hidden_tail = true;
  int max_n = 0, max_d = 0, max_q = 0;
  CtxLayout lay{};
  int ld = 0;
  int ptr_mode = PCABO_PTR_HOST;
  ModelState st;
  double *dX = nullptr, *dNoise = nullptr, *dF = nullptr, *dWeights = nullptr, *dWc = nullptr;
  long long* dRanks = nullptr;
  double *dDataMean = nullptr, *dPcaMean = nullptr, *dC = nullptr, *dLam = nullptr;
  double* dGbuf[2] = {nullptr, nullptr};
  double *dComps = nullptr, *dEvr = nullptr, *dZ = nullptr;
  double* dPcaOut = nullptr;
  double *dIn = nullptr, *hIn = nullptr;
  int *dK = nullptr, *dSweeps = nullptr, *dInfo = nullptr;
  double *dY = nullptr, *dYs = nullptr, *dYstats = nullptr, *dBounds4 = nullptr, *dZnMean = nullptr, *dUserNB = nullptr;
  double *dZnT = nullptr, *dAT = nullptr, *dNrm = nullptr, *dGram = nullptr, *dL = nullptr, *dR = nullptr;
  double *dTmp = nullptr, *dAlpha = nullptr, *dDiag = nullptr;
  double *dXq = nullptr, *dPartial = nullptr, *dVal = nullptr, *dGrad = nullptr, *dZq = nullptr, *dXout = nullptr;
  unsigned int* dCounters = nullptr;
  double* dKS = nullptr;
  double* dBestF = nullptr;
  double* dMll = nullptr;
  double* dArdLs = nullptr;
  double* dHyp = nullptr;
  char* dPostV = nullptr;
  char* dSample = nullptr;
  char *dRegion = nullptr, *hRegion = nullptr;
  bool in_batch = false; int batch_index = 0;
  HostMirror* hm = nullptr;
  double *hXq = nullptr, *hVal = nullptr, *hGrad = nullptr, *hSmall = nullptr, *hBestF = nullptr;
  double* hMll = nullptr;
  double* hArdLs = nullptr;
  double* hHyp = nullptr;
  MailPair* dMail = nullptr;
  bool mail_bar = false;
  MailPair* dPairs = nullptr;
  bool opt_resident = true;
  bool opt_group_acq = false;
  bool bestf_f32 = true;
  int srv_penalty = 0;
  unsigned long long seq = 0;
  OptCrew crew;
  bool registered = false;
  bool alone = true; int alone_age = 0;
  char err[512] = {0};
  bool prof = false;
  std::vector<ProfPair> pairs;
  size_t pairs_used = 0;
  double prof_ms[PROF_GROUPS] = {0};
  double prof_pair_ms = 0.0;
  double prof_empty_ms = 0.0;
  int64_t prof_launches[PROF_GROUPS] = {0};
  double prof_bytes[PROF_GROUPS] = {0}, prof_flops[PROF_GROUPS] = {0};
};

static std::mutex g_presence_mu;
static int g_presence_refs[64] = {0};
static void presence_path(char* buf, size_t n, int device, long pid) { snprintf(buf, n, "/dev/shm/pcabo.%d.%ld", device, pid); }
static void presence_register(int device) {
  if (device < 0 || device >= 64) return;
  std::lock_guard<std::mutex> lk(g_presence_mu);
  if (g_presence_refs[device]++ == 0) {
    char path[128]; presence_path(path, sizeof(path), device, (long)getpid());
    int fd = open(path, O_CREAT | O_WRONLY, 0644);
    if (fd >= 0) close(fd);
  }
}
static void presence_unregister(int device) {
  if (device < 0 || device >= 64) return;
  std::lock_guard<std::mutex> lk(g_presence_mu);
  if (g_presence_refs[device] > 0 && --g_presence_refs[device] == 0) {
    char path[128]; presence_path(path, sizeof(path), device, (long)getpid());
    unlink(path);
  }
}
static int presence_local_contexts(int device) {
  if (device < 0 || device >= 64) return 1;
  std::lock_guard<std::mutex> lk(g_presence_mu);
  return g_presence_refs[device];
}
static bool presence_alone(int device) {
  DIR* d = opendir("/dev/shm");
  if (!d) return true;
  char prefix[64]; snprintf(prefix, sizeof(prefix), "pcabo.%d.", device);
  const size_t pl = strlen(prefix);
  bool alone = true;
  while (struct dirent* e = readdir(d)) {
    if (strncmp(e->d_name, prefix, pl) != 0) continue;
    const long pid = atol(e->d_name + pl);
    if (pid <= 0 || pid == (long)getpid()) continue;
    if (kill((pid_t)pid, 0) == 0 || errno == EPERM) { alone = false; break; }
    char path[300]; snprintf(path, sizeof(path), "/dev/shm/%s", e->d_name);
    unlink(path);
  }
  closedir(d);
  return alone;
}

static int set_err(pcabo_ctx* c, int code, const char* fmt, const char* a = "", int v = 0) {
  if (c) snprintf(c->err, sizeof(c->err), fmt, a, v);
  if (c && (code == PCABO_ERR_TIMEOUT || code == PCABO_ERR_HIP)) c->st.launch_may_have_died();
  return code;
}
#define HIPCHK(call)                                                                         \
  do {                                                                                       \
    hipError_t e_ = (call);                                                                  \
    if (e_ != hipSuccess) return set_err(ctx, PCABO_ERR_HIP, "HIP error: %s (line %d)", hipGetErrorString(e_), __LINE__); \
  } while (0)

static hipError_t wait_stream(hipStream_t s) {
  const auto t0 = std::chrono::steady_clock::now();
  for (unsigned spins = 1;; ++spins) {
    hipError_t e = hipStreamQuery(s);
    if (e != hipErrorNotReady) return e == hipSuccess ? hipStreamSynchronize(s) : e;
    if ((spins & 63) == 0 && std::chrono::steady_clock::now() - t0 > std::chrono::milliseconds(2)) break;
    __builtin_ia32_pause();
  }
  return hipStreamSynchronize(s);
}
static hipError_t wait_event(hipEvent_t ev) {
  const auto t0 = std::chrono::steady_clock::now();
  for (unsigned spins = 1;; ++spins) {
    hipError_t e = hipEventQuery(ev);
    if (e != hipErrorNotReady) return e;
    if ((spins & 63) == 0 && std::chrono::steady_clock::now() - t0 > std::chrono::milliseconds(2)) break;
// ... 608 lines not shown
}

static int gp_fit_call(pcabo_ctx* ctx, const char* who, bool ard, const double* Z, const double* y, int n, int k,
                       const double* norm_bounds, int kernel, double* theta_inout, double* loss, int* info) {
  if (!ctx) return PCABO_ERR_ARG;
  if (!theta_inout) return set_err(ctx, PCABO_ERR_ARG, "%s: theta_inout is required", who);
  const double* unb = nullptr;
  int rc = stage_fit_inputs(ctx, who, ard, Z, y, n, k, norm_bounds, kernel, &unb);
  if (rc != PCABO_OK) return rc;
  std::vector<FitRun> run(1);
  run[0].init(theta_inout, ard ? k : 1, ard);
  run[0].bind(ctx->hMll);
  fit_rounds(run, n, [&](const std::vector<const double*>& th, int* st) { st[0] = mll_launch(ctx, ard, n, k, unb, th[0]); return (int)PCABO_OK; });
  const FitRun& r = run[0];
  if (r.status == PCABO_ERR_ARG) return theta_domain_err(ctx, who, ard);
  if (r.status != PCABO_OK) return r.status;
  memcpy(theta_inout, r.xr, (size_t)r.nvar * sizeof(double));
  if (loss) *loss = r.fr;
  if (info) r.report(info);
  return PCABO_OK;
}

int pcabo_gp_mll(pcabo_ctx* ctx, const double* Z, const double* y, int n, int k, const double* norm_bounds, int kernel,
                 const double* theta, double* loss, double* grad) {
  return gp_mll_call(ctx, "pcabo_gp_mll", false, Z, y, n, k, norm_bounds, kernel, theta, loss, grad);
}
int pcabo_gp_fit(pcabo_ctx* ctx, const double* Z, const double* y, int n, int k, const double* norm_bounds, int kernel,
                 double* theta_inout, double* loss, int* info) {
  return gp_fit_call(ctx, "pcabo_gp_fit", false, Z, y, n, k, norm_bounds, kernel, theta_inout, loss, info);
}
int pcabo_gp_mll_ard(pcabo_ctx* ctx, const double* Z, const double* y, int n, int k, const double* norm_bounds, int kernel,
                     const double* theta, double* loss, double* grad) {
  return gp_mll_call(ctx, "pcabo_gp_mll_ard", true, Z, y, n, k, norm_bounds, kernel, theta, loss, grad);
}
int pcabo_gp_fit_ard(pcabo_ctx* ctx, const double* Z, const double* y, int n, int k, const double* norm_bounds, int kernel,
                     double* theta_inout, double* loss, int* info) {
  return gp_fit_call(ctx, "pcabo_gp_fit_ard", true, Z, y, n, k, norm_bounds, kernel, theta_inout, loss, info);
}

int pcabo_acq_bounds(pcabo_ctx* ctx, double* bounds) {
  if (!ctx || !bounds) return PCABO_ERR_ARG;
  if (const int rc = collect_pending_wpca(ctx)) return rc;
  if (ctx->st.in_flight()) {
    HIPCHK(hipSetDevice(ctx->device));
    HIPCHK(wait_event(ctx->evBounds));
  } else if (!ctx->st.conditioned()) {
    return set_err(ctx, PCABO_ERR_ARG, "pcabo_acq_bounds: call pcabo_gp_condition first%s", "");
  }
  for (int c = 0; c < ctx->st.k; ++c) { bounds[c] = ctx->hm->acq_lo[c]; bounds[ctx->st.k + c] = ctx->hm->acq_hi[c]; }
  return PCABO_OK;
}

static const char* acq_arg_error(int acq, double scalar) {
  if (acq != PCABO_ACQ_LOG_EI && acq != PCABO_ACQ_PI && acq != PCABO_ACQ_UCB) return "unknown acquisition code";
  if (acq == PCABO_ACQ_UCB && !(std::isfinite(scalar) && scalar >= 0.0))
    return "PCABO_ACQ_UCB takes kappa = sqrt(beta) in the best_f slot: it must be finite and >= 0";
  return nullptr;
}

static AcqParams make_params(pcabo_ctx* ctx, double best_f, int maximize, int acq, int want_grad) {
  AcqParams p;
  p.best_f = ctx->bestf_f32 ? (double)(float)best_f : best_f;
  p.y_mean = 0.0; p.y_std = 1.0;
  p.inv_ls = 1.0 / ctx->st.lengthscale;
  p.maximize = maximize ? 1 : 0;
  p.acq = acq;
  p.kernel = ctx->st.kernel;
  p.want_grad = want_grad;
  return p;
}

static GpModel gp_model(const pcabo_ctx* c) { return {c->st.n, c->st.k, c->st.NP, c->ld, c->dZnT, c->dR, c->dAlpha, c->dBounds4, c->dYstats}; }
static GpArrays gp_arrays(const pcabo_ctx* c) { return {c->dZnMean, c->dL, c->dR, c->dZnT, c->dAT, c->dNrm, c->dYs}; }

static int acq_published(pcabo_ctx* ctx, FlagWait w) {
  if (w == FLAGS_UNPUBLISHED) {
    HIPCHK(hipGetLastError());
    return set_err(ctx, PCABO_ERR_TIMEOUT, "acquisition kernel finished without publishing its results%s", "");
  }
  if (w == FLAGS_LATE) return set_err(ctx, PCABO_ERR_TIMEOUT, "device did not publish acquisition results%s", "");
  return PCABO_OK;
}

static int eval_staged(pcabo_ctx* ctx, int nq, AcqParams& p, bool allow_gemm = true) {
  hipStream_t s = ctx->stream;
  const int k = ctx->st.k;
  const unsigned long long seq = ++ctx->seq;
  const QueryArgs* qa = nullptr;
  const double* xdev = nullptr;
  if ((size_t)nq * k <= PCABO_QA_MAX) {
    qa = reinterpret_cast<const QueryArgs*>(ctx->hXq);
  } else {
    HIPCHK(hipMemcpyAsync(ctx->dXq, ctx->hXq, (size_t)nq * k * sizeof(double), hipMemcpyHostToDevice, s));
    xdev = ctx->dXq;
  }
  const bool small = nq <= PCABO_INLAUNCH_MAXQ;
  if (!small && !p.want_grad && allow_gemm && score_gemm_possible(nq)) {
    if (!xdev) {
      HIPCHK(hipMemcpyAsync(ctx->dXq, ctx->hXq, (size_t)nq * k * sizeof(double), hipMemcpyHostToDevice, s));
      xdev = ctx->dXq;
    }
    ProfScope ps(ctx, 5, acq_bytes(ctx->st.n, k, nq, 0), acq_flops(ctx->st.n, k, nq, 0));
    launch_score(s, xdev, nq, gp_model(ctx), p, ctx->dKS, ctx->dPartial, ctx->dVal);
  } else {
    ProfScope ps(ctx, small ? 4 : 5, acq_bytes(ctx->st.n, k, nq, p.want_grad), acq_flops(ctx->st.n, k, nq, p.want_grad));
    launch_acq(s, qa, xdev, nq, gp_model(ctx), p, ctx->dPartial, ctx->dCounters, ctx->dVal, ctx->dGrad, small ? ctx->hVal : nullptr,
               small ? ctx->hGrad : nullptr, small ? ctx->hm : nullptr, seq);
  }
  if (!small) {
    HIPCHK(hipMemcpyAsync(ctx->hVal, ctx->dVal, (size_t)nq * sizeof(double), hipMemcpyDeviceToHost, s));
    if (p.want_grad) HIPCHK(hipMemcpyAsync(ctx->hGrad, ctx->dGrad, (size_t)nq * k * sizeof(double), hipMemcpyDeviceToHost, s));
    HIPCHK(wait_stream(s));
    HIPCHK(hipGetLastError());
    return PCABO_OK;
  }
  return acq_published(ctx, wait_flags(ctx->hm, 0, nq, seq, deadline_in(20), &s));
}

static int score_tail(pcabo_ctx* ctx, int nq, AcqParams& p) {
  hipStream_t s = ctx->stream;
  launch_score_tail(s, nq, gp_model(ctx), p, ctx->dKS, ctx->dPartial, ctx->dVal);
  HIPCHK(hipMemcpyAsync(ctx->hVal, ctx->dVal, (size_t)nq * sizeof(double), hipMemcpyDeviceToHost, s));
  HIPCHK(wait_stream(s));
  HIPCHK(hipGetLastError());
  return PCABO_OK;
}

struct GroupLaunches {
  int g0[8], gn[8], ng = 0;
  void add(int q0, int n) { g0[ng] = q0; gn[ng] = n; ++ng; }
};
static int eval_staged_groups(pcabo_ctx* ctx, const GroupLaunches& t, AcqParams& p) {
  hipStream_t s = ctx->stream;
  const unsigned long long seq = ++ctx->seq;
  const int *g0 = t.g0, *gn = t.gn, ng = t.ng;
  QueryArgs tab;
  unsigned* ent = reinterpret_cast<unsigned*>(tab.x);
  for (int g = 0; g < ng; ++g) ent[g] = ((unsigned)g0[g] << 8) | (unsigned)gn[g];
  {
    int nq = 0;
    for (int g = 0; g < ng; ++g) nq += gn[g];
    ProfScope ps(ctx, 4, acq_bytes(ctx->st.n, ctx->st.k, nq, p.want_grad), acq_flops(ctx->st.n, ctx->st.k, nq, p.want_grad));
    if (launch_acq_group(s, &tab, ng, ctx->hXq, gp_model(ctx), p, ctx->dPartial, ctx->dCounters + counters_group().start, ctx->dVal,
                         ctx->dGrad, ctx->hVal, ctx->hGrad, ctx->hm, seq, AcqBatch()) != 0)
      return set_err(ctx, PCABO_ERR_HIP, "the restart-group acquisition kernel could not be launched%s", "");
  }
  HIPCHK(hipGetLastError());
  const auto deadline = deadline_in(20);
  FlagWait w = FLAGS_SET;
  for (int g = 0; g < ng && w == FLAGS_SET; ++g) w = wait_flags(ctx->hm, g0[g], gn[g], seq, deadline, &s);
  return acq_published(ctx, w);
}
static bool group_mode(const pcabo_ctx* ctx, int q, int want_grad) {
  return ctx->opt_group_acq && want_grad && q <= PCABO_INLAUNCH_MAXQ && acq_group_possible(ctx->st.NP, ctx->st.k);
}

int pcabo_acq_eval(pcabo_ctx* ctx, const double* Xq, int q, double best_f, int maximize, int acq, double* val,
                   double* grad) {
  if (!ctx) return PCABO_ERR_ARG;
  if (!Xq || !val || q < 1 || q > ctx->max_q)
    return set_err(ctx, PCABO_ERR_ARG, "pcabo_acq_eval: bad argument or q beyond context capacity%s", "");
  if (const char* why = acq_arg_error(acq, best_f)) return set_err(ctx, PCABO_ERR_ARG, "pcabo_acq_eval: %s", why);
  if (!ctx->st.conditioned()) return set_err(ctx, PCABO_ERR_ARG, "pcabo_acq_eval: call pcabo_gp_condition first%s", "");
  HIPCHK(hipSetDevice(ctx->device));
  hipStream_t s = ctx->stream;
  const int k = ctx->st.k;
  const size_t nx = (size_t)q * k;
  if (ctx->ptr_mode == PCABO_PTR_HOST) memcpy(ctx->hXq, Xq, nx * sizeof(double));
  else {
    HIPCHK(hipMemcpyAsync(ctx->hXq, Xq, nx * sizeof(double), hipMemcpyDeviceToHost, s));
    HIPCHK(hipStreamSynchronize(s));
  }
  AcqParams p = make_params(ctx, best_f, maximize, acq, grad ? 1 : 0);
  int rc;
  if (group_mode(ctx, q, grad != nullptr) && ctx->ptr_mode == PCABO_PTR_HOST) {
    static_assert((PCABO_INLAUNCH_MAXQ + PCABO_GROUP_Q - 1) / PCABO_GROUP_Q <= 8, "GroupLaunches holds 8 groups");
    GroupLaunches t;
    for (int a = 0; a < q; a += PCABO_GROUP_Q) t.add(a, std::min(PCABO_GROUP_Q, q - a));
    rc = eval_staged_groups(ctx, t, p);
  } else {
    rc = eval_staged(ctx, q, p);
  }
  if (rc != PCABO_OK) return rc;
  if (ctx->ptr_mode == PCABO_PTR_HOST) {
    memcpy(val, ctx->hVal, (size_t)q * sizeof(double));
    if (grad) memcpy(grad, ctx->hGrad, nx * sizeof(double));
  } else {
    HIPCHK(hipMemcpyAsync(val, ctx->dVal, (size_t)q * sizeof(double), hipMemcpyDeviceToDevice, s));
    if (grad) HIPCHK(hipMemcpyAsync(grad, ctx->dGrad, nx * sizeof(double), hipMemcpyDeviceToDevice, s));
    HIPCHK(hipStreamSynchronize(s));
  }
  return PCABO_OK;
}

int pcabo_gp_condition_end_eval(pcabo_ctx* ctx, const double* Xq, int q, double best_f, int maximize, int acq,
                                double* val) {
  if (!ctx) return PCABO_ERR_ARG;
  if (!Xq || !val || q < 1 || q > ctx->max_q)
    return set_err(ctx, PCABO_ERR_ARG, "pcabo_gp_condition_end_eval: bad argument or q beyond context capacity%s", "");
  if (const char* why = acq_arg_error(acq, best_f)) return set_err(ctx, PCABO_ERR_ARG, "pcabo_gp_condition_end_eval: %s", why);
  if (!ctx->st.in_flight()) return set_err(ctx, PCABO_ERR_ARG, "pcabo_gp_condition_end_eval: no conditioning in flight%s", "");
  if (const int rc = collect_pending_wpca(ctx)) return rc;
  if (q <= PCABO_INLAUNCH_MAXQ || ctx->ptr_mode != PCABO_PTR_HOST) {
    int rc = pcabo_gp_condition_end(ctx);
    if (rc != PCABO_OK) return rc;
    return pcabo_acq_eval(ctx, Xq, q, best_f, maximize, acq, val, nullptr);
  }
  HIPCHK(hipSetDevice(ctx->device));
  memcpy(ctx->hXq, Xq, (size_t)q * ctx->st.k * sizeof(double));
  AcqParams p = make_params(ctx, best_f, maximize, acq, 0);
  const bool hidden = ctx->st.zn_consumed() && ctx->opt_hidden_tail && !ctx->prof && score_gemm_possible(q);
  int rc;
  if (hidden) {
    HIPCHK(hipStreamWaitEvent(ctx->stream2, ctx->evZn, 0));
    HIPCHK(hipMemcpyAsync(ctx->dXq, ctx->hXq, (size_t)q * ctx->st.k * sizeof(double), hipMemcpyHostToDevice, ctx->stream2));
    launch_score_ks_only(ctx->stream2, ctx->dXq, q, gp_model(ctx), p, ctx->dKS);
    HIPCHK(hipEventRecord(ctx->evKS, ctx->stream2));
    HIPCHK(hipStreamWaitEvent(ctx->stream, ctx->evKS, 0));
    rc = score_tail(ctx, q, p);
  } else {
    rc = eval_staged(ctx, q, p);
  }
  if (rc != PCABO_OK) { ctx->st.condition_failed(); return rc; }
  if (ctx->hm->chol_info != 0) {
    rc = pcabo_gp_condition_end(ctx);
    if (rc != PCABO_OK) return rc;
    rc = hidden ? score_tail(ctx, q, p) : eval_staged(ctx, q, p);
    if (rc != PCABO_OK) return rc;
  } else {
    ctx->st.condition_ended_ok(0.0);
  }
  memcpy(val, ctx->hVal, (size_t)q * sizeof(double));
  return PCABO_OK;
}

int pcabo_logei(pcabo_ctx* ctx, const double* Xq, int q, double best_f, int maximize, double* val, double* grad) {
  return pcabo_acq_eval(ctx, Xq, q, best_f, maximize, PCABO_ACQ_LOG_EI, val, grad);
}

struct BarMailbox {
  MailPair* m; const HostMirror* hm; int cap, k;
  void coords(int q0, int nq, const double* x, unsigned long long tag) const {
    for (int t = 0; t < nq * k; ++t) put_mail_pair(m + 1 + q0 * k + t, x[t], tag);
  }
  void controls(int q0, int nq, double what, unsigned long long tag) const {
    for (int j = 0; j < nq; ++j) put_mail_pair(m + 1 + cap * k + q0 + j, what, tag);
  }
  void flush() const { _mm_sfence(); }
  void post(int q0, int nq, const double* x, unsigned long long tag) const { coords(q0, nq, x, tag); controls(q0, nq, 1.0, tag); flush(); }
  unsigned long long tag_of(int q) const { return __atomic_load_n(&hm->qflag[q], __ATOMIC_ACQUIRE); }
  void leave(int q0, int nq, unsigned long long tag) const { controls(q0, nq, 0.0, tag); flush(); }
  void post_round(int nq, const double* xq, unsigned long long tag) const {
    coords(0, cap, xq, tag); controls(0, nq, 1.0, tag); controls(nq, cap - nq, 0.0, tag); flush();
  }
};

struct ResidentSession {
  pcabo_ctx* ctx; AcqParams& p;
  int cap = 0;
  BarMailbox mail() const { return BarMailbox{ctx->dMail, ctx->hm, cap, ctx->st.k}; }
  bool wanted(unsigned round_no, int nq) {
    if (round_no != 1) return false;
    if ((ctx->alone_age++ & 7) == 0) ctx->alone = presence_alone(ctx->device);
    if (ctx->srv_penalty > 0) { --ctx->srv_penalty; return false; }
    return ctx->opt_resident && ctx->mail_bar && !ctx->opt_group_acq && ctx->alone && presence_local_contexts(ctx->device) == 1 &&
           !ctx->prof && acq_server_possible(nq, ctx->st.n, ctx->st.k, ctx->st.NP);
  }
  int start(int nq) {
    cap = nq;
    launch_acq(ctx->stream, nullptr, nullptr, cap, gp_model(ctx), p, ctx->dPartial, ctx->dCounters, ctx->dVal, ctx->dGrad,
               ctx->hVal, ctx->hGrad, ctx->hm, ctx->seq + 1, ctx->dMail, ctx->dPairs);
    HIPCHK(hipGetLastError());
    return PCABO_OK;
  }
  int round(int nq, bool first) {
    const auto now = [] { return std::chrono::duration<double>(std::chrono::steady_clock::now().time_since_epoch()).count(); };
    const unsigned long long tag = ++ctx->seq;
    const double tp = now();
    mail().post_round(nq, ctx->hXq, tag);
    if (wait_flags(ctx->hm, 0, nq, tag, deadline_in(3)) != FLAGS_SET) {
      (void)set_err(ctx, PCABO_ERR_TIMEOUT, "resident acquisition kernel did not answer%s", "");
      stop();
      ctx->srv_penalty = 1000;
      return eval_staged(ctx, nq, p);
    }
    if (first && now() - tp > 1e-3) ctx->srv_penalty = 40;
    return PCABO_OK;
  }
  int pair(CrewCall& crew, RunRestarts& run) {
    const unsigned long long seq0 = ctx->seq;
    BarMailbox mb = mail();
    const FreePair fp = free_pair(crew, run, mb, seq0);
    HIPCHK(hipStreamSynchronize(ctx->stream));
    ctx->seq = seq0 + std::max(fp.used[0], fp.used[1]) + 1;
    cap = 0;
    if (fp.got_nan[0] || fp.got_nan[1]) return set_err(ctx, PCABO_ERR_NAN, "NaN in acquisition gradient%s", "");
    if (fp.timed_out[0] || fp.timed_out[1]) ctx->srv_penalty = 1000;
    else if (fp.slow_first[0] || fp.slow_first[1]) ctx->srv_penalty = 40;
    return PCABO_OK;
  }
  void stop() {
    if (cap <= 0) return;
    mail().post_round(0, ctx->hXq, ++ctx->seq);
    (void)hipStreamSynchronize(ctx->stream);
    cap = 0;
  }
  ~ResidentSession() { stop(); }
};

int pcabo_optimize_acqf(pcabo_ctx* ctx, const double* ics, int num_restarts, int batch_limit, const double* bounds,
                        int maxiter, double best_f, int maximize, int acq, double* cand, double* vals, int* info,
                        int* failed) {
  if (!ctx) return PCABO_ERR_ARG;
  if (!ics || !bounds || !cand || !vals || num_restarts < 1 || batch_limit < 1 || num_restarts > ctx->max_q)
    return set_err(ctx, PCABO_ERR_ARG, "pcabo_optimize_acqf: bad argument%s", "");
  if (const char* why = acq_arg_error(acq, best_f)) return set_err(ctx, PCABO_ERR_ARG, "pcabo_optimize_acqf: %s", why);
  if (!ctx->st.conditioned()) return set_err(ctx, PCABO_ERR_ARG, "pcabo_optimize_acqf: call pcabo_gp_condition first%s", "");
  HIPCHK(hipSetDevice(ctx->device));
  const int k = ctx->st.k;
  RunRestarts run;
  run.init(ics, bounds, num_restarts, batch_limit, k, maxiter);
  run.bind(ctx->hXq, ctx->hVal, ctx->hGrad);
  std::vector<RestartGroup>& grp = run.grp;
  const int ngroups = (int)grp.size();
  AcqParams p = make_params(ctx, best_f, maximize, acq, 1);
  std::vector<char> pending(ngroups, 0);
  std::vector<int> qoff(ngroups, -1);
  CrewCall crew(ctx->crew, run, pending);
  ResidentSession srv{ctx, p};
  for (unsigned round_no = 1;; ++round_no) {
    crew.advance_all();
    const int nq = pack_active(run, qoff);
    if (nq == 0) break;
    int rc;
    if (srv.wanted(round_no, nq)) {
      if ((rc = srv.start(nq)) != PCABO_OK) return rc;
      if (ngroups == 2 && grp[0].active && grp[1].active && nq == num_restarts) {
        if ((rc = srv.pair(crew, run)) != PCABO_OK) return rc;
        if (!grp[0].active && !grp[1].active) break;
        continue;
      }
    }
    if (srv.cap > 0) {
      rc = srv.round(nq, round_no == 1);
    } else if (group_mode(ctx, nq, 1) && batch_limit <= PCABO_GROUP_Q && ngroups <= 8) {
      GroupLaunches t;
      for (int gi = 0; gi < ngroups; ++gi) if (qoff[gi] >= 0) t.add(qoff[gi], grp[gi].nq);
      rc = eval_staged_groups(ctx, t, p);
    } else {
      rc = eval_staged(ctx, nq, p);
    }
    if (rc != PCABO_OK) return rc;
    if (!absorb_packed(run, qoff)) return set_err(ctx, PCABO_ERR_NAN, "NaN in acquisition gradient%s", "");
  }
  srv.stop();
  const bool redo = run.end_points(cand, vals) > 0;
  const bool any_failed = run.report(info, 0);
  if (redo) {
    AcqParams pv = make_params(ctx, best_f, maximize, acq, 0);
    memcpy(ctx->hXq, cand, (size_t)num_restarts * k * sizeof(double));
    int rc = eval_staged(ctx, num_restarts, pv, false);
    if (rc != PCABO_OK) return rc;
    for (int j = 0; j < num_restarts; ++j) vals[j] = ctx->hVal[j];
  }
  if (failed) *failed = any_failed;
  return PCABO_OK;
}

int pcabo_inverse_map(pcabo_ctx* ctx, const double* z, double* x) {
  if (!ctx || !z || !x) return PCABO_ERR_ARG;
  if (!ctx->st.have_wpca) return set_err(ctx, PCABO_ERR_ARG, "pcabo_inverse_map: call pcabo_wpca first%s", "");
  if (!ctx->in_batch && ctx->opt_hidden_tail) {
    if (const int rc = collect_pending_wpca(ctx)) return rc;
    const double* h = small_at(ctx, small_wpca(ctx->lay.s));
    const PcaParts pp = pca_parts(ctx->lay.s);
    inverse_map_host(z, h + pp.comps, h + pp.pca_mean, h + pp.data_mean, ctx->st.k, ctx->st.d, x);
    return PCABO_OK;
  }
  HIPCHK(hipSetDevice(ctx->device));
  hipStream_t s = ctx->stream;
  memcpy(ctx->hXq, z, (size_t)ctx->st.k * sizeof(double));
  const unsigned long long seq = ++ctx->seq;
  double* hx = small_at(ctx, small_imap_x(ctx->lay.s));
  launch_inverse_map(s, ctx->hXq, ctx->dComps, ctx->dDataMean, ctx->dPcaMean, ctx->st.k, ctx->st.d, ctx->dXout, nullptr, ZB(),
                     hx, ctx->hm, seq);
  HIPCHK(hipGetLastError());
  const FlagWait w = wait_flags(ctx->hm, 0, 1, seq, deadline_in(20), &s);
  if (w == FLAGS_UNPUBLISHED) {
    HIPCHK(hipGetLastError());
    return set_err(ctx, PCABO_ERR_TIMEOUT, "inverse-map kernel finished without publishing its result%s", "");
  }
  if (w == FLAGS_LATE) return set_err(ctx, PCABO_ERR_TIMEOUT, "device did not publish the inverse map%s", "");
  memcpy(x, hx, (size_t)ctx->st.d * sizeof(double));
  return PCABO_OK;
}

int pcabo_get_gp_state(pcabo_ctx* ctx, double* K_chol, double* Rinv, double* alpha, double* y_mean_std,
                       double* norm_bounds) {
  if (!ctx) return PCABO_ERR_ARG;
  if (!ctx->st.holds_factors()) return set_err(ctx, PCABO_ERR_ARG, "pcabo_get_gp_state: call pcabo_gp_condition first%s", "");
  HIPCHK(hipSetDevice(ctx->device));
  hipStream_t s = ctx->stream;
  const size_t n = ctx->st.rows_held(), w = n * sizeof(double), pitch = (size_t)ctx->ld * sizeof(double);
  if (K_chol) HIPCHK(hipMemcpy2DAsync(K_chol, w, ctx->dL, pitch, w, n, hipMemcpyDeviceToHost, s));
  if (Rinv) HIPCHK(hipMemcpy2DAsync(Rinv, w, ctx->dR, pitch, w, n, hipMemcpyDeviceToHost, s));
  if (alpha) HOST_OUT(alpha, ctx->dAlpha, n, double);
  HIPCHK(hipStreamSynchronize(s));
  if (y_mean_std) { y_mean_std[0] = ctx->hm->y_mean; y_mean_std[1] = ctx->hm->y_std; }
  if (norm_bounds)
    for (int c = 0; c < ctx->st.k; ++c) { norm_bounds[c] = ctx->hm->norm_lo[c]; norm_bounds[ctx->st.k + c] = ctx->hm->norm_hi[c]; }
  return PCABO_OK;
}

int pcabo_get_gram(pcabo_ctx* ctx, double* K) {
  if (!ctx || !K) return PCABO_ERR_ARG;
  if (!ctx->st.conditioned()) return set_err(ctx, PCABO_ERR_ARG, "pcabo_get_gram: call pcabo_gp_condition first%s", "");
  HIPCHK(hipSetDevice(ctx->device));
  const size_t n = ctx->st.n, w = n * sizeof(double), pitch = (size_t)ctx->ld * sizeof(double);
  ctx->st.gram_fetched();
  launch_gram(ctx->stream, ctx->dAT, ctx->dNrm, ctx->st.n, ctx->st.NP, round_up(ctx->st.k, 4), ctx->ld, ctx->st.noise, ctx->st.kernel, ctx->dGram,
              nullptr, nullptr, nullptr);
  HIPCHK(hipMemcpy2DAsync(K, w, ctx->dGram, pitch, w, n, hipMemcpyDeviceToHost, ctx->stream));
  HIPCHK(hipStreamSynchronize(ctx->stream));
  for (size_t i = 0; i < n; ++i)
    for (size_t j = i + 1; j < n; ++j) K[i * n + j] = K[j * n + i];
  return PCABO_OK;
}


int pcabo_set_profiling(pcabo_ctx* ctx, int enabled) {
  if (!ctx) return PCABO_ERR_ARG;
  HIPCHK(hipSetDevice(ctx->device));
  if (enabled && ctx->pairs.empty()) {
    ctx->pairs.resize(PROF_POOL);
    for (auto& p : ctx->pairs) { HIPCHK(hipEventCreate(&p.a)); HIPCHK(hipEventCreate(&p.b)); p.group = 0; }
  }
  if (!enabled) prof_resolve(ctx);
  if (enabled && !ctx->prof) {
    prof_resolve(ctx);
    double med[2] = {0.0, 0.0};
    for (int mode = 0; mode < 2; ++mode) {
      std::vector<float> r;
      for (int i = 0; i < 64; ++i) {
        HIPCHK(hipEventRecord(ctx->pairs[i].a, ctx->stream));
        if (mode == 1) hipLaunchKernelGGL(k_nop, dim3(1), dim3(64), 0, ctx->stream);
        HIPCHK(hipEventRecord(ctx->pairs[i].b, ctx->stream));
      }
      HIPCHK(hipStreamSynchronize(ctx->stream));
      for (int i = 0; i < 64; ++i) { float ms = 0.f; if (hipEventElapsedTime(&ms, ctx->pairs[i].a, ctx->pairs[i].b) == hipSuccess) r.push_back(ms); }
      if (!r.empty()) { std::sort(r.begin(), r.end()); med[mode] = r[r.size() / 2]; }
// ... 1706 lines not shown
```

para-ortho-pca-bo_amd/pcabo/_native.py:

```python
from __future__ import annotations

import ctypes as C
import math
import os
from typing import Optional

import numpy as np

ABI_VERSION = 2
KERNEL_MATERN52, KERNEL_RBF = 0, 1
ACQ_LOG_EI, ACQ_PI, ACQ_UCB = 0, 1, 2
PTR_HOST, PTR_DEVICE = 0, 1
OPT_RESIDENT, OPT_BESTF_F32, OPT_GROUP_ACQ, OPT_DEVICE_LBFGSB = 0, 1, 2, 3
OPT_HIDDEN_TAIL = 5
POST_OBS_NOISE = 1
EXTEND_BELIEVER = 1
POST_CENTRED = 2
POST_MAX_SAMPLES = 1024
FIT_THETA0 = (0.006737946999085467, 0.0, 0.0)
FIT_TASK_NOT_PD = -2
PROFILE_GROUPS = ("wpca", "gram", "cholesky", "root_inverse_alpha", "acq_partial", "acq_large_batches")

HW_QUEUES_ENV, HW_QUEUES_WANTED = "GPU_MAX_HW_QUEUES", 16


def hw_queues_advice(streams: int) -> Optional[str]:
    try:
        have = int(os.environ.get(HW_QUEUES_ENV, "4"))
    except ValueError:
        have = 4
    if have >= streams:
        return None
    return (f"{HW_QUEUES_ENV}={os.environ.get(HW_QUEUES_ENV, 'unset (default 4)')}: {streams} streams of this batch will share "
            f"hardware queues and their kernels serialise; set {HW_QUEUES_ENV}={max(HW_QUEUES_WANTED, streams)} in the environment "
            "before the process makes its first GPU call")


_LIB_PATH = os.path.join(os.path.dirname(os.path.abspath(__file__)), "..", "lib", "libpcabo.so")

EXPORTS = [
    "pcabo_abi_version", "pcabo_device_count", "pcabo_ctx_create", "pcabo_ctx_destroy",
    "pcabo_set_pointer_mode", "pcabo_set_option", "pcabo_last_error", "pcabo_wpca", "pcabo_gp_condition", "pcabo_gp_condition_begin",
    "pcabo_gp_condition_end", "pcabo_gp_condition_end_eval", "pcabo_wpca_gp_condition_begin", "pcabo_wpca_results",
    "pcabo_gp_mll", "pcabo_gp_fit", "pcabo_gp_mll_ard", "pcabo_gp_fit_ard",
    "pcabo_acq_bounds",
    "pcabo_acq_eval", "pcabo_logei", "pcabo_gp_posterior", "pcabo_batch_gp_posterior", "pcabo_gp_posterior_sample", "pcabo_batch_gp_posterior_sample", "pcabo_gp_loo", "pcabo_batch_gp_loo",
    "pcabo_gp_extend", "pcabo_gp_truncate", "pcabo_gp_extended",
    "pcabo_batch_gp_extend", "pcabo_batch_gp_truncate", "pcabo_batch_gp_extended", "pcabo_optimize_acqf", "pcabo_inverse_map", "pcabo_get_gp_state",
    "pcabo_get_gram", "pcabo_lbfgsb_minimize", "pcabo_lbfgsb_set_vector_kernels", "pcabo_lbfgsb_set_sum_order", "pcabo_sobol_scramble", "pcabo_sobol_draw", "pcabo_sobol_draw_rows", "pcabo_torch_randint2", "pcabo_torch_multinomial_rows", "pcabo_boltzmann_pick_rows", "pcabo_set_profiling",
    "pcabo_get_profile", "pcabo_get_profile_calibration", "pcabo_reset_profile",
    "pcabo_batch_create", "pcabo_batch_destroy", "pcabo_batch_last_error", "pcabo_batch_ctx",
    "pcabo_batch_wpca_gp_condition_begin", "pcabo_batch_wpca_results", "pcabo_batch_acq_bounds",
    "pcabo_batch_acq_score", "pcabo_batch_acq_score_begin", "pcabo_batch_acq_score_end",
    "pcabo_batch_gp_condition_end_eval", "pcabo_batch_optimize_acqf", "pcabo_batch_inverse_map", "pcabo_batch_device_acq_eval",
    "pcabo_batch_busy", "pcabo_batch_gp_condition_end_eval_begin", "pcabo_batch_gp_condition_end_eval_end",
    "pcabo_batch_optimize_acqf_begin", "pcabo_batch_optimize_acqf_end", "pcabo_batch_inverse_map_begin", "pcabo_batch_inverse_map_end",
    "pcabo_batch_set_input_strides", "pcabo_batch_gp_condition_begin",
    "pcabo_batch_gp_mll", "pcabo_batch_gp_fit", "pcabo_batch_gp_fit_rounds", "pcabo_batch_gp_mll_ard", "pcabo_batch_gp_fit_ard",
    "pcabo_batch_set_profiling", "pcabo_batch_get_profile", "pcabo_batch_set_active", "pcabo_batch_set_workers", "pcabo_batch_set_option",
    "pcabo_device_lbfgsb_limits",
    "pcabo_bbob_table_doubles", "pcabo_bbob_create", "pcabo_bbob_destroy", "pcabo_bbob_eval", "pcabo_bbob_eval_many",
    "pcabo_comm_unique_id", "pcabo_comm_create", "pcabo_gather_best", "pcabo_comm_last_error", "pcabo_comm_destroy",
]


class PcaboError(RuntimeError):
    def __init__(self, code: int, msg: str):
        super().__init__(f"libpcabo error {code}: {msg}")
        self.code = code


def lib_path() -> str:
    return os.path.normpath(os.environ.get("PCABO_LIB") or _LIB_PATH)


def _load() -> C.CDLL:
    path = lib_path()
    if not os.path.exists(path):
        raise ImportError(
            f"{path} not found: build it with `python -c 'import __graft_entry__ as g; g.build()'` "
            "(or `make -C para-ortho-pca-bo_amd/csrc`).  There is no CPU fallback for the HIP path.")
    lib = C.CDLL(path)
    lib.pcabo_abi_version.restype = C.c_int
    if lib.pcabo_abi_version() != ABI_VERSION:
        raise ImportError(f"{path}: ABI version mismatch")
    dp, ip, vp = C.POINTER(C.c_double), C.POINTER(C.c_int), C.c_void_p
    lib.pcabo_device_count.restype = C.c_int
    lib.pcabo_ctx_create.argtypes = [C.c_int, C.c_int, C.c_int, C.c_int, C.POINTER(vp)]
    lib.pcabo_ctx_destroy.argtypes = [vp]
    lib.pcabo_set_pointer_mode.argtypes = [vp, C.c_int]
    lib.pcabo_set_option.argtypes = [vp, C.c_int, C.c_int]
    lib.pcabo_last_error.argtypes = [vp, C.c_char_p, C.c_int]
    lib.pcabo_wpca.argtypes = [vp, vp, vp, vp, C.c_int, C.c_int, C.c_int, C.c_double, C.c_int, vp,
                               vp, vp, vp, vp, ip, vp]
    lib.pcabo_gp_condition.argtypes = [vp, vp, vp, C.c_int, C.c_int, vp, C.c_double, C.c_double, C.c_int]
    lib.pcabo_gp_condition_begin.argtypes = lib.pcabo_gp_condition.argtypes
    lib.pcabo_gp_condition_end.argtypes = [vp]
    lib.pcabo_gp_mll.argtypes = [vp, vp, vp, C.c_int, C.c_int, vp, C.c_int, vp, dp, vp]
    lib.pcabo_gp_fit.argtypes = [vp, vp, vp, C.c_int, C.c_int, vp, C.c_int, vp, dp, vp]
    lib.pcabo_gp_mll_ard.argtypes = lib.pcabo_gp_mll.argtypes
    lib.pcabo_gp_fit_ard.argtypes = lib.pcabo_gp_fit.argtypes
    lib.pcabo_wpca_results.argtypes = [vp, vp, vp, vp, vp, ip]
    lib.pcabo_gp_condition_end_eval.argtypes = [vp, vp, C.c_int, C.c_double, C.c_int, C.c_int, vp]
    lib.pcabo_wpca_gp_condition_begin.argtypes = [vp, vp, vp, vp, C.c_int, C.c_int, C.c_int, C.c_double, C.c_int, vp,
                                                  vp, C.c_double, C.c_double, C.c_int, vp, vp, vp, vp, ip]
    lib.pcabo_acq_bounds.argtypes = [vp, vp]
    lib.pcabo_acq_eval.argtypes = [vp, vp, C.c_int, C.c_double, C.c_int, C.c_int, vp, vp]
    lib.pcabo_logei.argtypes = [vp, vp, C.c_int, C.c_double, C.c_int, vp, vp]
    lib.pcabo_gp_posterior.argtypes = [vp, vp, C.c_int, C.c_int, vp, vp, vp]
    lib.pcabo_batch_gp_posterior.argtypes = [vp, vp, C.c_int, C.c_int, vp, vp, vp, vp]
    lib.pcabo_gp_posterior_sample.argtypes = [vp, vp, C.c_int, C.c_int, vp, C.c_int, vp, vp, dp]
    lib.pcabo_batch_gp_posterior_sample.argtypes = [vp, vp, C.c_int, C.c_int, vp, C.c_int, vp, vp, vp, vp]
    lib.pcabo_gp_loo.argtypes = [vp, vp, vp, vp, vp, dp]
    lib.pcabo_batch_gp_loo.argtypes = [vp, vp, vp, vp, vp, vp, vp]
    lib.pcabo_gp_extend.argtypes = [vp, vp, vp, C.c_int, C.c_int]
    lib.pcabo_gp_truncate.argtypes = [vp, C.c_int]
    lib.pcabo_gp_extended.argtypes = [vp, ip, ip]
    lib.pcabo_batch_gp_extend.argtypes = [vp, vp, vp, C.c_int, C.c_int, vp]
    lib.pcabo_batch_gp_truncate.argtypes = [vp, C.c_int, vp]
    lib.pcabo_batch_gp_extended.argtypes = [vp, ip, ip]
    lib.pcabo_optimize_acqf.argtypes = [vp, vp, C.c_int, C.c_int, vp, C.c_int, C.c_double, C.c_int, C.c_int,
                                        vp, vp, vp, ip]
    lib.pcabo_inverse_map.argtypes = [vp, vp, vp]
    lib.pcabo_get_gp_state.argtypes = [vp, vp, vp, vp, vp, vp]
    lib.pcabo_get_gram.argtypes = [vp, vp]
    lib.pcabo_sobol_scramble.argtypes = [vp, vp, C.c_int]
    lib.pcabo_sobol_draw.argtypes = [vp, vp, C.c_int, C.c_int, vp, vp, vp]
    lib.pcabo_sobol_draw_rows.argtypes = [vp, vp, vp, C.c_int, C.c_int, vp, C.c_longlong, vp]
    lib.pcabo_set_profiling.argtypes = [vp, C.c_int]
    lib.pcabo_get_profile.argtypes = [vp, C.c_int, dp, C.POINTER(C.c_int64), dp, dp]
    lib.pcabo_reset_profile.argtypes = [vp]
    lib.pcabo_get_profile_calibration.argtypes = [vp, dp, dp]
    lib.pcabo_lbfgsb_set_vector_kernels.argtypes = [C.c_int]
    lib.pcabo_batch_create.argtypes = [C.c_int, C.c_int, C.c_int, C.c_int, C.c_int, C.POINTER(vp)]
    lib.pcabo_comm_unique_id.argtypes = [C.c_char_p]
    lib.pcabo_comm_create.argtypes = [C.c_char_p, C.c_int, C.c_int, C.c_int, C.POINTER(vp)]
    lib.pcabo_gather_best.argtypes = [vp, vp, C.c_int, vp]
    lib.pcabo_comm_last_error.argtypes = [vp, C.c_char_p, C.c_int]
    lib.pcabo_comm_destroy.argtypes = [vp]
    lib.pcabo_batch_destroy.argtypes = [vp]
    lib.pcabo_batch_set_workers.argtypes = [vp, C.c_int]
    lib.pcabo_batch_set_option.argtypes = [vp, C.c_int, C.c_int]
    lib.pcabo_batch_last_error.argtypes = [vp, C.c_char_p, C.c_int]
    lib.pcabo_batch_ctx.argtypes = [vp, C.c_int]
    lib.pcabo_batch_wpca_gp_condition_begin.argtypes = [vp, vp, vp, vp, vp, C.c_int, C.c_int, C.c_int, C.c_double, C.c_int,
                                                        C.c_double, C.c_double, C.c_int]
    lib.pcabo_batch_wpca_results.argtypes = [vp, vp, vp, vp, vp, vp]
    lib.pcabo_batch_acq_bounds.argtypes = [vp, vp]
    lib.pcabo_batch_gp_condition_end_eval.argtypes = [vp, vp, C.c_int, vp, C.c_int, C.c_int, vp, vp]
    lib.pcabo_batch_optimize_acqf.argtypes = [vp, vp, C.c_int, C.c_int, vp, C.c_int, vp, C.c_int, C.c_int, vp, vp, vp, vp, vp]
    lib.pcabo_batch_inverse_map.argtypes = [vp, vp, vp]
    lib.pcabo_batch_device_acq_eval.argtypes = [vp, vp, C.c_int, vp, C.c_int, C.c_int, vp, vp]
    lib.pcabo_batch_busy.argtypes = [vp]
    lib.pcabo_batch_gp_condition_end_eval_begin.argtypes = [vp, vp, C.c_int, vp, C.c_int, C.c_int]
    lib.pcabo_batch_gp_condition_end_eval_end.argtypes = [vp, vp, C.c_int, vp, C.c_int, C.c_int, vp, vp]
    lib.pcabo_batch_acq_score.argtypes = [vp, vp, C.c_int, vp, C.c_int, C.c_int, vp, vp]
    lib.pcabo_batch_acq_score_begin.argtypes = [vp, vp, C.c_int, vp, C.c_int, C.c_int]
    lib.pcabo_batch_acq_score_end.argtypes = [vp, C.c_int, vp, vp]
    lib.pcabo_batch_optimize_acqf_begin.argtypes = [vp, vp, C.c_int, C.c_int, vp, C.c_int, vp, C.c_int, C.c_int]
    lib.pcabo_batch_optimize_acqf_end.argtypes = [vp, C.c_int, C.c_int, vp, vp, vp, vp, vp]
    lib.pcabo_batch_inverse_map_begin.argtypes = [vp, vp]
    lib.pcabo_batch_set_input_strides.argtypes = [vp, C.c_size_t, C.c_size_t, C.c_size_t]
    lib.pcabo_batch_gp_condition_begin.argtypes = [vp, vp, vp, C.c_int, C.c_int, vp, C.c_double, C.c_double, C.c_int]
    lib.pcabo_batch_inverse_map_end.argtypes = [vp, vp]
    lib.pcabo_batch_set_profiling.argtypes = [vp, C.c_int]
    lib.pcabo_batch_set_active.argtypes = [vp, vp]
    lib.pcabo_batch_get_profile.argtypes = [vp, vp]
    lib.pcabo_batch_gp_mll.argtypes = [vp, vp, vp, vp, vp]
    lib.pcabo_batch_gp_fit.argtypes = [vp, vp, vp, vp, vp]
    lib.pcabo_batch_gp_fit_rounds.argtypes = [vp]
    lib.pcabo_batch_gp_mll_ard.argtypes = [vp, vp, C.c_int, vp, vp, vp]
    lib.pcabo_batch_gp_fit_ard.argtypes = [vp, vp, C.c_int, vp, vp, vp]
    for name in EXPORTS:
        getattr(lib, name).restype = C.c_int
    lib.pcabo_batch_ctx.restype = vp
    return lib


LIB = _load()
FG_CALLBACK = C.CFUNCTYPE(C.c_double, C.POINTER(C.c_double), C.POINTER(C.c_double), C.c_void_p)
LIB.pcabo_lbfgsb_minimize.argtypes = [
    C.c_int, C.c_void_p, C.c_void_p, C.c_void_p, FG_CALLBACK, C.c_void_p, C.c_int, C.c_double, C.c_double,
    C.c_int, C.c_int, C.c_int, C.POINTER(C.c_double), C.POINTER(C.c_int), C.POINTER(C.c_int), C.POINTER(C.c_int)]


LIB.pcabo_debug_lbfgsb_branch_names.argtypes = [C.c_char_p, C.c_int]
LIB.pcabo_debug_lbfgsb_branches.argtypes = [C.c_void_p, C.c_int]


def _branch_names():
    buf = C.create_string_buffer(2048)
    count = LIB.pcabo_debug_lbfgsb_branch_names(buf, 2048)
    names = tuple(buf.value.decode().split(","))
    assert len(names) == count
    return names


LBFGSB_BRANCHES = _branch_names()
DEVICE_GROUP_FIELDS = ("niter", "nfev", "warnflag", "task", "status", "evaluations", "ties", "evaluation_cap")
if hasattr(LIB, "pcabo_debug_batch_lbfgsb_branches"):
    LIB.pcabo_debug_batch_lbfgsb_branches.argtypes = [C.c_void_p, C.c_void_p, C.c_int]
    LIB.pcabo_debug_batch_lbfgsb_device_out.argtypes = [C.c_void_p, C.c_void_p, C.c_int]


def device_count() -> int:
# ... 205 lines not shown
                                                  _ptr(val)))
        self._keep = None
        return val

    def acq_bounds(self) -> np.ndarray:
        b = np.empty((2, self.k))
        self._chk(LIB.pcabo_acq_bounds(self._h, _ptr(b)))
        return b

    def acq_eval(self, Xq, best_f, maximize=False, acq=ACQ_LOG_EI, grad=True):
        Xq = _f64(Xq).reshape(-1, self.k)
        q = Xq.shape[0]
        val = np.empty(q)
        g = np.empty((q, self.k)) if grad else None
        self._chk(LIB.pcabo_acq_eval(self._h, _ptr(Xq), q, float(best_f), int(bool(maximize)), int(acq), _ptr(val),
                                     _ptr(g)))
        return (val, g) if grad else val

    def gp_posterior(self, Xq, observation_noise=False, covariance=False) -> dict:
        Xq = _f64(Xq).reshape(-1, self.k)
        q = Xq.shape[0]
        mean, var = np.empty(q), np.empty(q)
        cov = np.empty((q, q)) if covariance else None
        self._chk(LIB.pcabo_gp_posterior(self._h, _ptr(Xq), q, POST_OBS_NOISE if observation_noise else 0, _ptr(mean), _ptr(var),
                                         _ptr(cov)))
        out = {"mean": mean, "variance": var}
        if covariance:
            out["covariance"] = cov
        return out

    def gp_posterior_samples(self, Xq, n_samples=None, base_samples=None, seed=None, observation_noise=False, centred=False) -> dict:
        Xq = _f64(Xq).reshape(-1, self.k)
        q = Xq.shape[0]
        base = sample_base(q, n_samples, base_samples, seed)
        S = base.shape[0]
        samples, mean = np.empty((S, q)), np.empty(q)
        jitter = C.c_double(0.0)
        flags = (POST_OBS_NOISE if observation_noise else 0) | (POST_CENTRED if centred else 0)
        self._chk(LIB.pcabo_gp_posterior_sample(self._h, _ptr(Xq), q, flags, _ptr(base), S, _ptr(samples), _ptr(mean),
                                                C.byref(jitter)))
        return {"samples": samples, "mean": mean, "jitter": float(jitter.value)}

    def gp_loo(self) -> dict:
        n = self.n
        mean, var, z, lpd = np.empty(n), np.empty(n), np.empty(n), np.empty(n)
        total = C.c_double(0.0)
        self._chk(LIB.pcabo_gp_loo(self._h, _ptr(mean), _ptr(var), _ptr(z), _ptr(lpd), C.byref(total)))
        return {"mean": mean, "variance": var, "z": z, "lpd": lpd, "lpd_sum": float(total.value)}

    def gp_extend(self, Zp, y=None) -> int:
        Zp = _f64(Zp).reshape(-1, self.k)
        p = Zp.shape[0]
        yv = None if y is None else _f64(y, (p,))
        self._chk(LIB.pcabo_gp_extend(self._h, _ptr(Zp), _ptr(yv), p, EXTEND_BELIEVER if y is None else 0))
        self.n += p
        return self.n

    def gp_truncate(self, n0=None) -> int:
        n0 = self.n_base if n0 is None else int(n0)
        self._chk(LIB.pcabo_gp_truncate(self._h, n0))
        self.n = n0
        return self.n

    @property
    def n_base(self) -> int:
        nb, n = C.c_int(0), C.c_int(0)
        self._chk(LIB.pcabo_gp_extended(self._h, C.byref(nb), C.byref(n)))
        return int(nb.value)

    def optimize_acqf(self, ics, bounds, best_f, maximize=False, acq=ACQ_LOG_EI, batch_limit=5, maxiter=200):
        ics = _f64(ics).reshape(-1, self.k)
        nr = ics.shape[0]
        bounds = _f64(bounds, (2, self.k))
        cand = np.empty((nr, self.k))
        vals = np.empty(nr)
        ng = (nr + batch_limit - 1) // batch_limit
        info = np.zeros((ng, 4), dtype=np.int32)
        failed = C.c_int(0)
        self._chk(LIB.pcabo_optimize_acqf(self._h, _ptr(ics), nr, int(batch_limit), _ptr(bounds), int(maxiter),
                                          float(best_f), int(bool(maximize)), int(acq), _ptr(cand), _ptr(vals),
                                          _ptr(info), C.byref(failed)))
        return cand, vals, info, bool(failed.value)

    def inverse_map(self, z) -> np.ndarray:
        z = _f64(z).reshape(-1)
        x = np.empty(self.d)
        self._chk(LIB.pcabo_inverse_map(self._h, _ptr(z), _ptr(x)))
        return x

    def gp_state(self):
        n, k = self.n, self.k
        L, R, alpha, ys, nb = np.empty((n, n)), np.empty((n, n)), np.empty(n), np.empty(2), np.empty((2, k))
        self._chk(LIB.pcabo_get_gp_state(self._h, _ptr(L), _ptr(R), _ptr(alpha), _ptr(ys), _ptr(nb)))
        return {"L": np.tril(L), "R": np.tril(R), "alpha": alpha, "y_mean": ys[0], "y_std": ys[1], "norm_bounds": nb}

    def gram(self) -> np.ndarray:
        K = np.empty((self.n, self.n))
        self._chk(LIB.pcabo_get_gram(self._h, _ptr(K)))
        return K

    def set_profiling(self, on: bool) -> None:
        self._chk(LIB.pcabo_set_profiling(self._h, int(bool(on))))

    def reset_profile(self) -> None:
        self._chk(LIB.pcabo_reset_profile(self._h))

    def profile(self) -> dict:
        out = {}
        for i, name in enumerate(PROFILE_GROUPS):
            ms, cnt, by, fl = C.c_double(0), C.c_int64(0), C.c_double(0), C.c_double(0)
            self._chk(LIB.pcabo_get_profile(self._h, i, C.byref(ms), C.byref(cnt), C.byref(by), C.byref(fl)))
            out[name] = {"ms": ms.value, "launches": cnt.value, "bytes": by.value, "flops": fl.value}
        return out

    def profile_calibration(self) -> dict:
        a, b = C.c_double(0), C.c_double(0)
        self._chk(LIB.pcabo_get_profile_calibration(self._h, C.byref(a), C.byref(b)))
        return {"pair_ms": a.value, "empty_kernel_ms": b.value}


class _BorrowedContext(Context):

    def __init__(self, handle, max_n, max_d, max_q, device):
        self._h = C.c_void_p(handle)
        self.max_n, self.max_d, self.max_q, self.device = max_n, max_d, max_q, device
        self.n = self.d = self.k = 0

    def close(self) -> None:
        self._h = C.c_void_p()


class Batch:

    def __init__(self, B: int, max_n: int, max_d: int, max_q: int = 512, device: int = 0, workers: int = 0,
                 group_acq: bool = True, device_lbfgsb: int = 0):
        self._h = C.c_void_p()
        rc = LIB.pcabo_batch_create(int(device), int(B), int(max_n), int(max_d), int(max_q), C.byref(self._h))
        if rc != 0:
            msg = self._err() if self._h else "no usable HIP device (the HIP path has no CPU fallback)"
            if self._h:
                LIB.pcabo_batch_destroy(self._h)
                self._h = C.c_void_p()
            raise PcaboError(rc, msg)
        self.B, self.max_n, self.max_d, self.max_q, self.device = B, max_n, max_d, max_q, device
        self.n = self.d = 0
        self.k = np.zeros(B, dtype=np.int32)
        self.ctx = [_BorrowedContext(LIB.pcabo_batch_ctx(self._h, b), max_n, max_d, max_q, device) for b in range(B)]
        if workers:
            self.set_workers(workers)
        if not group_acq:
            self._chk(LIB.pcabo_batch_set_option(self._h, OPT_GROUP_ACQ, 0))
        if device_lbfgsb:
            self._chk(LIB.pcabo_batch_set_option(self._h, OPT_DEVICE_LBFGSB, int(device_lbfgsb)))
        self.device_lbfgsb = int(device_lbfgsb)
        advice = hw_queues_advice(min(B, int(workers) if workers else 8) + 2)
        if advice:
            import warnings
            warnings.warn(advice, RuntimeWarning, stacklevel=2)

    def set_workers(self, workers: int) -> None:
        self._chk(LIB.pcabo_batch_set_workers(self._h, int(workers)))

    def _err(self) -> str:
        buf = C.create_string_buffer(512)
        LIB.pcabo_batch_last_error(self._h, buf, 512)
        return buf.value.decode(errors="replace")
# ... 519 lines not shown
```

para-ortho-pca-bo_amd/pcabo/acqopt.py:

```python
from __future__ import annotations

import warnings
from time import perf_counter
from typing import Optional

import numpy as np

from . import _native
from . import initializers as _init


ALLOWED_ACQUISITION_FUNCTION_STRINGS = (
    "expected_improvement",
    "probability_of_improvement",
    "upper_confidence_bound",
)
ALLOWED_SHORTHAND_ACQUISITION_FUNCTION_STRINGS = {
    "EI": "expected_improvement",
    "PI": "probability_of_improvement",
    "UCB": "upper_confidence_bound",
}


def acquisition_long_name(name: str, odd_name: str = "Oddly defined name") -> str:
    name = name.strip()
    if name in ALLOWED_SHORTHAND_ACQUISITION_FUNCTION_STRINGS:
        return ALLOWED_SHORTHAND_ACQUISITION_FUNCTION_STRINGS[name]
    if name.lower() in ALLOWED_ACQUISITION_FUNCTION_STRINGS:
        return name
    raise ValueError(odd_name.format(name=name))


def ucb_kappa(beta) -> float:
    import torch
    return float(torch.as_tensor(float(beta)).sqrt())


def checked_ucb_beta(ucb_beta, acquisition_name: str) -> Optional[float]:
    if ucb_beta is None:
        return None
    beta = float(ucb_beta)
    if not (np.isfinite(beta) and beta >= 0.0):
        raise ValueError(f"ucb_beta must be finite and >= 0, got {ucb_beta!r}")
    if acquisition_name.strip().lower() not in ("ucb", "upper_confidence_bound"):
        raise ValueError(f"ucb_beta is the parameter of the upper-confidence-bound acquisition; it was given together with "
                         f"{acquisition_name!r}")
    return beta


Q_STRATEGIES = ("kriging_believer", "constant_liar_min", "constant_liar_mean", "constant_liar_max")


def checked_q(q, q_strategy):
    if isinstance(q, bool) or not isinstance(q, (int, np.integer)) or q < 1:
        raise ValueError(f"q must be an integer >= 1, got {q!r}")
    if q_strategy not in Q_STRATEGIES:
        raise ValueError(f"q_strategy must be one of {', '.join(Q_STRATEGIES)}; got {q_strategy!r}")
    return int(q), q_strategy


def liar_value(strategy: str, f_evals) -> float:
    f = np.asarray(f_evals, dtype=np.float64)
    return float({"constant_liar_min": f.min, "constant_liar_mean": f.mean, "constant_liar_max": f.max}[strategy]())


def moved_scalar(s, v, maximize: bool, acq_code: int):
    if acq_code == _native.ACQ_UCB:
        return s
    return max(s, v) if maximize else min(s, v)


def optimize_acqf(ctx: "_native.Context", bounds: np.ndarray, best_f: float, maximize: bool, acq_code: int,
                  num_restarts: int, raw_samples: int, batch_limit: int = 5, maxiter: int = 200, engine=None,
                  breakdown: Optional[dict] = None, trace: Optional[dict] = None, raw: Optional[np.ndarray] = None,
                  raw_vals: Optional[np.ndarray] = None, before_lbfgsb=None):
    pb = breakdown if breakdown is not None else {}
    engines = [engine] if engine is not None and raw is None else []
    ready = [raw] if raw is not None else []
    ready_vals = [raw_vals] if raw is not None and raw_vals is not None else []

    def initial_conditions():
        t0 = perf_counter()
        raw = ready.pop() if ready else _init.draw_sobol(bounds, raw_samples, engines.pop() if engines else None)
        t1 = perf_counter()
        vals = ready_vals.pop() if ready_vals else ctx.acq_eval(raw, best_f, maximize, acq_code, grad=False)
        t2 = perf_counter()
        if acq_code == _native.ACQ_PI:
            idx = _init.initialize_q_batch_nonneg(vals, num_restarts)
        else:
            idx = _init.initialize_q_batch(vals, num_restarts)
        t3 = perf_counter()
        pb["sobol"] = pb.get("sobol", 0.0) + t1 - t0
        pb["raw_eval"] = pb.get("raw_eval", 0.0) + t2 - t1
        pb["init_pick"] = pb.get("init_pick", 0.0) + t3 - t2
        if trace is not None:
            trace.update(raw_vals=vals.copy(), ic_idx=np.asarray(idx).copy())
        return raw[idx]

    ics = initial_conditions()
    if before_lbfgsb is not None:
        before_lbfgsb()
    t_opt = perf_counter()
    cand, vals, info, failed = ctx.optimize_acqf(ics, bounds, best_f, maximize, acq_code, batch_limit=batch_limit,
                                                 maxiter=maxiter)
    pb["lbfgsb"] = pb.get("lbfgsb", 0.0) + perf_counter() - t_opt
    if failed:
        warnings.warn("Optimization failed in `gen_candidates_scipy`; trying again with a new set of "
                      "initial conditions.", RuntimeWarning)
        if trace is not None:
            trace["retried"] = True
        ics = initial_conditions()
        cand, vals, info, failed = ctx.optimize_acqf(ics, bounds, best_f, maximize, acq_code,
                                                     batch_limit=batch_limit, maxiter=maxiter)
    best = int(np.argmax(vals))
    if trace is not None:
        trace.update(ics=ics.copy(), cands=cand.copy(), vals=vals.copy(), chosen=best, info=info.copy(),
                     k=int(cand.shape[1]))
    return cand[best].reshape(1, -1), cand, vals, info


def propose(ctx: "_native.Context", bounds: np.ndarray, best_f: float, maximize: bool, acq_code: int, num_restarts: int,
            raw_samples: int, batch_limit: int = 5, maxiter: int = 200, q_eff: int = 1, strategy: str = "kriging_believer",
            f_evals=None, breakdown: Optional[dict] = None, trace: Optional[dict] = None, raw: Optional[np.ndarray] = None,
            raw_vals: Optional[np.ndarray] = None, before_lbfgsb=None):
    believer = strategy == "kriging_believer"
    if strategy not in Q_STRATEGIES:
        raise ValueError(f"q_strategy must be one of {', '.join(Q_STRATEGIES)}; got {strategy!r}")
    liar = None if believer or q_eff <= 1 else liar_value(strategy, f_evals)
    s, n0, cands, infos = best_f, None, [], []
    try:
        z, _, _, info = optimize_acqf(ctx, bounds, s, maximize, acq_code, num_restarts, raw_samples, batch_limit, maxiter,
                                      breakdown=breakdown, trace=trace, raw=raw, raw_vals=raw_vals, before_lbfgsb=before_lbfgsb)
        cands.append(z)
        infos.append(info)
        for _ in range(1, q_eff):
            v = float(ctx.gp_posterior(z)["mean"][0]) if believer else liar
            n = ctx.n
            ctx.gp_extend(z, None if believer else [v])
            n0 = n if n0 is None else n0
            s = moved_scalar(s, v, maximize, acq_code)
            tr = None
            if trace is not None:
                tr = {"best_f": s, "believed": v}
                trace.setdefault("proposals", []).append(tr)
            z, _, _, info = optimize_acqf(ctx, bounds, s, maximize, acq_code, num_restarts, raw_samples, batch_limit, maxiter,
                                          breakdown=breakdown, trace=tr)
            cands.append(z)
            infos.append(info)
    finally:
        if n0 is not None:
            ctx.gp_truncate(n0)
    return np.concatenate(cands, axis=0), infos
```

Measured before the change: 400.7 BO iterations/s.

## Fuse raw scoring, Boltzmann initial-condition pick and L-BFGS-B into one native call

```diff
diff --git a/include/pcabo.h b/include/pcabo.h
--- a/include/pcabo.h
+++ b/include/pcabo.h
@@ -94,6 +94,12 @@
 int pcabo_optimize_acqf(pcabo_ctx* ctx, const double* ics, int num_restarts, int batch_limit,
                         const double* bounds, int maxiter, double best_f, int maximize, int acq,
                         double* cand, double* vals, int* info, int* failed);
+
+enum { PCABO_PROPOSE_NO_WAKE = 1 };
+int pcabo_propose_acqf(pcabo_ctx* ctx, const double* raw, int n_raw, void* blob, double eta, int num_restarts, int batch_limit,
+                       const double* bounds, int maxiter, double best_f, int maximize, int acq, int flags, double* raw_vals,
+                       int64_t* ic_idx, double* ics, double* cand, double* vals, int* info, int* failed, int* picked,
+                       double* phase_seconds);
 
 int pcabo_inverse_map(pcabo_ctx* ctx, const double* z, double* x);
 
diff --git a/para-ortho-pca-bo_amd/Algorithms/BayesianOptimization/DeviceBayesianOptimizer.py b/para-ortho-pca-bo_amd/Algorithms/BayesianOptimization/DeviceBayesianOptimizer.py
--- a/para-ortho-pca-bo_amd/Algorithms/BayesianOptimization/DeviceBayesianOptimizer.py
+++ b/para-ortho-pca-bo_amd/Algorithms/BayesianOptimization/DeviceBayesianOptimizer.py
@@ -83,6 +83,7 @@
         self._record_trace = bool(kwargs.pop("record_trace", False))
         self._guard = RunGuard(kwargs.pop("torch_threads", 4), kwargs.pop("gc_freeze", True))
         self._resident = bool(kwargs.pop("resident", True))
+        self._one_call = bool(kwargs.pop("one_call", _acqopt.one_call_default()))
         self._fantasy_points = int(kwargs.pop("fantasy_points", 0))
         if self._fantasy_points < 0:
             raise ValueError("fantasy_points must be >= 0")
@@ -169,6 +170,10 @@
             print(self.FINAL_LINE)
         self.restore_random_states()
 
+    def _scores_in_one_call(self, acq) -> bool:
+        cfg = self._torch_config
+        return self._one_call and _acqopt.one_call_applies(self._ctx, acq.acq_code, cfg["NUM_RESTARTS"], cfg["RAW_SAMPLES"])
+
     def _q_eff(self) -> int:
         return max(1, min(self._q, self.budget - len(self.f_evals)))
 
diff --git a/para-ortho-pca-bo_amd/Algorithms/BayesianOptimization/PCA_BO.py b/para-ortho-pca-bo_amd/Algorithms/BayesianOptimization/PCA_BO.py
--- a/para-ortho-pca-bo_amd/Algorithms/BayesianOptimization/PCA_BO.py
+++ b/para-ortho-pca-bo_amd/Algorithms/BayesianOptimization/PCA_BO.py
@@ -240,7 +240,10 @@
         raw = _init.draw_sobol(bounds, raw_samples, engine)
         self.phase_breakdown["sobol"] = self.phase_breakdown.get("sobol", 0.0) + perf_counter() - t0
         raw_vals = None
-        if self.__gp_pending and self.__early_scoring:
+        one_call = self._scores_in_one_call(acq)
+        if self.__gp_pending and self.__early_scoring and one_call:
+            self.__gp_pending = False
+        elif self.__gp_pending and self.__early_scoring:
             t0 = perf_counter()
             raw_vals = ctx.gp_wait_eval(raw, acq.device_scalar, acq.maximize, acq.acq_code)
             self.__gp_pending = False
@@ -252,7 +255,7 @@
             ctx, bounds, acq.device_scalar, acq.maximize, acq.acq_code, num_restarts, raw_samples, batch_limit, 200,
             q_eff=self._q_eff(), strategy=self._q_strategy, f_evals=self.f_evals,
             raw=raw, raw_vals=raw_vals, breakdown=self.phase_breakdown,
-            trace=self.trace[-1] if self._record_trace else None,
+            trace=self.trace[-1] if self._record_trace else None, one_call=one_call,
             before_lbfgsb=self._prefetch_noise)
         self.timing_logs["optimize_acqf"].append(perf_counter() - start)
         self.lbfgsb_info.extend(infos)
diff --git a/para-ortho-pca-bo_amd/Algorithms/BayesianOptimization/Vanilla_BO.py b/para-ortho-pca-bo_amd/Algorithms/BayesianOptimization/Vanilla_BO.py
--- a/para-ortho-pca-bo_amd/Algorithms/BayesianOptimization/Vanilla_BO.py
+++ b/para-ortho-pca-bo_amd/Algorithms/BayesianOptimization/Vanilla_BO.py
@@ -49,14 +49,15 @@
         engine = _init.scrambled_sobol_engine(self.dimension)
         raw = _init.draw_sobol(self.__box, cfg["RAW_SAMPLES"], engine)
         raw_vals = None
-        if not self._fit_gp:
+        one_call = self._scores_in_one_call(acq)
+        if not self._fit_gp and not one_call:
             t0 = perf_counter()
             raw_vals = ctx.gp_wait_eval(raw, acq.device_scalar, acq.maximize, acq.acq_code)
             self.phase_breakdown["raw_eval"] = self.phase_breakdown.get("raw_eval", 0.0) + perf_counter() - t0
         new_x, infos = _acqopt.propose(
             ctx, self.__box, acq.device_scalar, acq.maximize, acq.acq_code, cfg["NUM_RESTARTS"], cfg["RAW_SAMPLES"], 5, 200,
             q_eff=self._q_eff(), strategy=self._q_strategy, f_evals=self.f_evals, raw=raw, raw_vals=raw_vals, breakdown=self.phase_breakdown,
-            trace=self.trace[-1] if self._record_trace else None)
+            trace=self.trace[-1] if self._record_trace else None, one_call=one_call)
         self.timing_logs["optimize_acqf"].append(perf_counter() - start)
         self.lbfgsb_info.extend(infos)
         return new_x
diff --git a/para-ortho-pca-bo_amd/csrc/host_entry.cpp b/para-ortho-pca-bo_amd/csrc/host_entry.cpp
--- a/para-ortho-pca-bo_amd/csrc/host_entry.cpp
+++ b/para-ortho-pca-bo_amd/csrc/host_entry.cpp
@@ -1,4 +1,5 @@
 #include "../../include/pcabo.h"
+#include "host_side.h"
 #include "lbfgsb.h"
 
 #include <algorithm>
@@ -156,12 +157,15 @@
     out[i] = (int64_t)(y & 1u);
   }
 }
+inline bool mt_blob_ok(const TorchMt* s) {
+  return s->seeded && s->left >= 1 && s->left <= 624 && (s->left == 1 || (s->next <= 624 && s->next + (uint64_t)s->left <= 625));
+}
 }
 
 int pcabo_torch_randint2(void* blob, int64_t count, int64_t* out) {
   if (!blob || !out || count < 0) return PCABO_ERR_ARG;
   TorchMt* s = static_cast<TorchMt*>(blob);
-  if (!s->seeded || s->left < 1 || s->left > 624 || s->next > 624) return PCABO_ERR_ARG;
+  if (!mt_blob_ok(s)) return PCABO_ERR_ARG;
   while (count > 0) {
     int64_t take;
     if (s->left == 1) {
@@ -183,14 +187,16 @@
 }
 
 namespace {
-void multinomial_row(TorchMt* s, const double* w, int n, int n_pick, double* ratio, int* best, int64_t* out) {
+void draw_variates(TorchMt* s, int n, double* q) {
   for (int i = 0; i < n; ++i) {
     const uint64_t hi = mt_draw(s), lo = mt_draw(s);
     const uint64_t r64 = (hi << 32) | lo;
     const double u = (double)(r64 & ((1ull << 53) - 1)) * 1.1102230246251565e-16;
-    const double q = -std::log1p(-u);
-    ratio[i] = w[i] / q;
-  }
+    q[i] = -std::log1p(-u);
+  }
+}
+void top_ratios(const double* w, const double* q, int n, int n_pick, double* ratio, int* best, int64_t* out) {
+  for (int i = 0; i < n; ++i) ratio[i] = w[i] / q[i];
   int have = 0;
   for (int i = 0; i < n; ++i) {
     const double v = ratio[i];
@@ -200,41 +206,68 @@
     best[pos] = i;
     if (have < n_pick) ++have;
   }
+  if (out) for (int j = 0; j < n_pick; ++j) out[j] = best[j];
+}
+void pick_from_variates(const double* v, const double* q, int n, int n_pick, double eta, double* w, double* ratio, int* best,
+                        int64_t* out, int* flag) {
+  double mean = 0.0, m2 = 0.0;
+  int arg = 0;
+  for (int i = 0; i < n; ++i) {
+    const double d = v[i] - mean;
+    mean += d / (double)(i + 1);
+    m2 += d * (v[i] - mean);
+    if (v[i] > v[arg]) arg = i;
+  }
+  const double sd = std::sqrt(m2 / (double)(n - 1));
+  if (!(sd > 0.0)) { *flag = 1; return; }
+  double scale = eta;
+  for (;;) {
+    bool inf = false;
+    for (int i = 0; i < n; ++i) { w[i] = std::exp(scale * ((v[i] - mean) / sd)); inf = inf || std::isinf(w[i]); }
+    if (!inf) break;
+    scale *= 0.5;
+  }
+  top_ratios(w, q, n, n_pick, ratio, best, nullptr);
+  for (int j = 0; j + 1 < n_pick; ++j)
+    if (ratio[best[j]] == ratio[best[j + 1]]) { *flag = 1; return; }
+  int at_edge = 0;
+  for (int i = 0; i < n; ++i) at_edge += ratio[i] == ratio[best[n_pick - 1]];
+  if (at_edge > 1) { *flag = 1; return; }
   for (int j = 0; j < n_pick; ++j) out[j] = best[j];
-}
-}
+  bool has = false;
+  for (int j = 0; j < n_pick; ++j) has = has || out[j] == arg;
+  if (!has) out[n_pick - 1] = arg;
+  *flag = 0;
+}
+}
+
+}
+
+bool torch_blob_ok(const void* blob) { return blob && mt_blob_ok(static_cast<const TorchMt*>(blob)); }
+AheadPick::AheadPick(int n_, int n_pick_)
+    : n(n_), n_pick(n_pick_), before(sizeof(TorchMt)), q((size_t)n_), w((size_t)n_), ratio((size_t)n_), best((size_t)n_pick_) {}
+void AheadPick::draw(void* blob_) {
+  blob = blob_;
+  memcpy(before.data(), blob, sizeof(TorchMt));
+  draw_variates(static_cast<TorchMt*>(blob), n, q.data());
+}
+void AheadPick::put_back() { if (blob) memcpy(blob, before.data(), sizeof(TorchMt)); }
+int AheadPick::pick(const double* vals, double eta, int64_t* out) {
+  int flag = 1;
+  pick_from_variates(vals, q.data(), n, n_pick, eta, w.data(), ratio.data(), best.data(), out, &flag);
+  if (flag == 1) put_back();
+  return flag;
+}
+
+extern "C" {
 
 namespace {
 void boltzmann_rows(void* const* blobs, const double* vals, int r0, int r1, int n, int n_pick, double eta, int64_t* out, int* flags) {
-  std::vector<double> w((size_t)n), ratio((size_t)n);
-  std::vector<int> best((size_t)n_pick);
+  AheadPick ahead(n, n_pick);
   for (int r = r0; r < r1; ++r) {
-    TorchMt* s = static_cast<TorchMt*>(blobs[r]);
-    if (!s) { flags[r] = 2; continue; }
-    const double* v = vals + (size_t)r * n;
-    double mean = 0.0, m2 = 0.0;
-    int arg = 0;
-    for (int i = 0; i < n; ++i) {
-      const double d = v[i] - mean;
-      mean += d / (double)(i + 1);
-      m2 += d * (v[i] - mean);
-      if (v[i] > v[arg]) arg = i;
-    }
-    const double sd = std::sqrt(m2 / (double)(n - 1));
-    if (!(sd > 0.0)) { flags[r] = 1; continue; }
-    double scale = eta;
-    for (;;) {
-      bool inf = false;
-      for (int i = 0; i < n; ++i) { w[i] = std::exp(scale * ((v[i] - mean) / sd)); inf = inf || std::isinf(w[i]); }
-      if (!inf) break;
-      scale *= 0.5;
-    }
-    int64_t* o = out + (size_t)r * n_pick;
-    multinomial_row(s, w.data(), n, n_pick, ratio.data(), best.data(), o);
-    bool has = false;
-    for (int j = 0; j < n_pick; ++j) has = has || o[j] == arg;
-    if (!has) o[n_pick - 1] = arg;
-    flags[r] = 0;
+    if (!blobs[r]) { flags[r] = 2; continue; }
+    ahead.draw(blobs[r]);
+    flags[r] = ahead.pick(vals + (size_t)r * n, eta, out + (size_t)r * n_pick);
   }
 }
 }
@@ -243,23 +276,36 @@
   if (!blobs || !vals || !out || !flags || rows < 1 || n < 2 || n_pick < 1 || n_pick > n) return PCABO_ERR_ARG;
   for (int r = 0; r < rows; ++r) {
     const TorchMt* s = static_cast<const TorchMt*>(blobs[r]);
-    if (s && (!s->seeded || s->left < 1 || s->left > 624 || s->next > 624)) return PCABO_ERR_ARG;
+    if (s && !mt_blob_ok(s)) return PCABO_ERR_ARG;
   }
   boltzmann_rows(blobs, vals, 0, rows, n, n_pick, eta, out, flags);
+  return PCABO_OK;
+}
+
+int pcabo_debug_boltzmann_two_halves(void* blob, const double* vals, int n, int n_pick, double eta, int put_back, int64_t* out, int* flag) {
+  if (!vals || !out || !flag || n < 2 || n_pick < 1 || n_pick > n || !torch_blob_ok(blob)) return PCABO_ERR_ARG;
+  AheadPick ahead(n, n_pick);
+  ahead.draw(blob);
+  if (put_back) {
+    ahead.put_back();
+    ahead.draw(blob);
+  }
+  *flag = ahead.pick(vals, eta, out);
   return PCABO_OK;
 }
 
 int pcabo_torch_multinomial_rows(void* const* blobs, const double* weights, int rows, int n, int n_pick, int64_t* out) {
   if (!blobs || !weights || !out || rows < 1 || n < 1 || n_pick < 1 || n_pick > n) return PCABO_ERR_ARG;
-  std::vector<double> ratio((size_t)n);
+  std::vector<double> ratio((size_t)n), q((size_t)n);
   std::vector<int> best((size_t)n_pick);
   for (int r = 0; r < rows; ++r) {
     TorchMt* s = static_cast<TorchMt*>(blobs[r]);
     if (!s) continue;
-    if (!s->seeded || s->left < 1 || s->left > 624 || s->next > 624) return PCABO_ERR_ARG;
-    multinomial_row(s, weights + (size_t)r * n, n, n_pick, ratio.data(), best.data(), out + (size_t)r * n_pick);
-  }
-  return PCABO_OK;
-}
-
-}
+    if (!mt_blob_ok(s)) return PCABO_ERR_ARG;
+    draw_variates(s, n, q.data());
+    top_ratios(weights + (size_t)r * n, q.data(), n, n_pick, ratio.data(), best.data(), out + (size_t)r * n_pick);
+  }
+  return PCABO_OK;
+}
+
+}
diff --git a/para-ortho-pca-bo_amd/csrc/host_selftest.cpp b/para-ortho-pca-bo_amd/csrc/host_selftest.cpp
--- a/para-ortho-pca-bo_amd/csrc/host_selftest.cpp
+++ b/para-ortho-pca-bo_amd/csrc/host_selftest.cpp
@@ -128,6 +128,64 @@
   for (int j = 0; j < n_pick; ++j) CHECK(idx[j] >= 0 && idx[j] < n && idx[n_pick + j] == -1 && idx[2 * n_pick + j] >= 0, "multinomial pick %d", j);
   blobs[3].left = 900;
   CHECK(pcabo_torch_randint2(&blobs[3], 4, bits.data()) == PCABO_ERR_ARG, "a broken blob accepted");
+
+  for (int r : {0, 5, 11, 12}) {
+    std::vector<double> row(vals.begin() + (size_t)r * n, vals.begin() + (size_t)(r + 1) * n);
+    if (r == 12) row[100] = NAN;
+    Blob two = again[r], rows1 = again[r];
+    const Blob before = two;
+    std::vector<int64_t> a(n_pick, -1), b(n_pick, -1);
+    int flag1 = -1;
+    void* p1 = &rows1;
+    CHECK(pcabo_boltzmann_pick_rows(&p1, row.data(), 1, n, n_pick, 1.0, b.data(), &flag1) == PCABO_OK, "pick row %d again", r);
+    CHECK(torch_blob_ok(&two), "blob of row %d refused", r);
+    AheadPick ahead(n, n_pick);
+    ahead.draw(&two);
+    CHECK(memcmp(&two, &before, sizeof(Blob)) != 0, "the draw of row %d left its generator alone", r);
+    ahead.put_back();
+    CHECK(memcmp(&two, &before, sizeof(Blob)) == 0, "put_back of row %d", r);
+    ahead.draw(&two);
+    const int flag = ahead.pick(row.data(), 1.0, a.data());
+    CHECK(flag == flag1 && flag == (r == 5 || r == 12 ? 1 : 0), "flag of the two halves on row %d: %d / %d", r, flag, flag1);
+    if (flag == 1) {
+      CHECK(memcmp(&two, &before, sizeof(Blob)) == 0, "the two halves moved the generator of a row without spread (row %d)", r);
+      CHECK(memcmp(&rows1, &before, sizeof(Blob)) == 0, "a row without spread moved its generator (row %d)", r);
+      for (int j = 0; j < n_pick; ++j) CHECK(a[j] == -1, "a row without spread wrote pick %d", j);
+    } else {
+      for (int j = 0; j < n_pick; ++j) CHECK(a[j] == b[j], "row %d pick %d: the two halves differ from the one call", r, j);
+      CHECK(memcmp(&two, &rows1, sizeof(Blob)) == 0, "generator of row %d after the two halves", r);
+    }
+  }
+  struct { int left, seeded; uint64_t next; bool ok; } shapes[] = {
+      {1, 1, 0, true}, {1, 1, 9999, true}, {624, 1, 1, true}, {624, 1, 2, false}, {2, 1, 623, true}, {2, 1, 624, false},
+      {0, 1, 0, false}, {625, 1, 0, false}, {300, 0, 10, false}, {300, 1, 325, true}, {300, 1, 326, false},
+      {300, 1, ~0ull - 298, false} , {2, 1, ~0ull, false}, {624, 1, ~0ull - 622, false}, {1, 1, ~0ull, true}};
+  for (const auto& sh : shapes) {
+    Blob t = again[1];
+    t.left = sh.left; t.seeded = sh.seeded; t.next = sh.next;
+    void* pt = &t;
+    int fl = -1;
+    CHECK(torch_blob_ok(&t) == sh.ok, "checker on left %d next %llu", sh.left, (unsigned long long)sh.next);
+    if (sh.ok) continue;
+    CHECK(pcabo_torch_randint2(&t, 4, bits.data()) == PCABO_ERR_ARG, "randint2 took left %d next %llu", sh.left, (unsigned long long)sh.next);
+    CHECK(pcabo_boltzmann_pick_rows(&pt, vals.data(), 1, n, n_pick, 1.0, out1.data(), &fl) == PCABO_ERR_ARG, "pick rows took left %d", sh.left);
+    CHECK(pcabo_torch_multinomial_rows(&pt, w.data(), 1, n, n_pick, idx.data()) == PCABO_ERR_ARG, "multinomial rows took left %d", sh.left);
+  }
+  CHECK(!torch_blob_ok(nullptr), "a null blob accepted");
+}
+
+void test_helper_wake() {
+  OptCrew crew;
+  { OptCrew::Awake a(crew); }
+  for (int rep = 0; rep < 3; ++rep) {
+    OptCrew::Awake a(crew);
+    std::atomic<int> ran{0};
+    crew.helper.begin([&] { ran.fetch_add(1); });
+    CHECK(ran.load() == 0, "the helper ran before it was asked");
+    for (int i = 1; i <= 5; ++i) { crew.helper.wait(crew.helper.post()); CHECK(ran.load() == i, "round %d ran %d times", i, ran.load()); }
+    crew.helper.end();
+  }
+  crew.shutdown();
 }
 
 void test_sobol_rows() {
@@ -1166,6 +1224,7 @@
   test_sobol();
   test_sobol_rows();
   test_torch_rng();
+  test_helper_wake();
   test_plan();
   test_restart_group();
   test_crew();
diff --git a/para-ortho-pca-bo_amd/csrc/host_side.h b/para-ortho-pca-bo_amd/csrc/host_side.h
--- a/para-ortho-pca-bo_amd/csrc/host_side.h
+++ b/para-ortho-pca-bo_amd/csrc/host_side.h
@@ -15,6 +15,21 @@
 #include <thread>
 #include <utility>
 #include <vector>
+
+constexpr size_t TORCH_BLOB_BYTES = 5056;
+bool torch_blob_ok(const void* blob);
+struct AheadPick {
+  AheadPick(int n, int n_pick);
+  void draw(void* blob);
+  int pick(const double* vals, double eta, int64_t* out);
+  void put_back();
+ private:
+  int n, n_pick;
+  void* blob = nullptr;
+  std::vector<unsigned char> before;
+  std::vector<double> q, w, ratio;
+  std::vector<int> best;
+};
 
 struct RestartGroup : LbfgsbDriver {
   int q0 = 0, nq = 0, k = 0;
@@ -138,6 +153,7 @@
     cv.notify_one();
   }
   void end() { active.store(false, std::memory_order_release); }
+  void wake() { if (!active.load(std::memory_order_acquire)) begin([] {}); }
   void shutdown() {
     if (!th.joinable()) return;
     { std::lock_guard<std::mutex> lk(mu); quit.store(true, std::memory_order_release); active.store(false, std::memory_order_release); }
@@ -155,6 +171,12 @@
 struct OptCrew {
   OptHelper helper;
   std::vector<std::unique_ptr<OptHelper>> more;
+  struct Awake {
+    OptHelper& h;
+    explicit Awake(OptCrew& c) : h(c.helper) { h.wake(); }
+    Awake(const Awake&) = delete;
+    ~Awake() { h.end(); }
+  };
   void shutdown() {
     helper.shutdown();
     for (auto& h : more) h->shutdown();
diff --git a/para-ortho-pca-bo_amd/csrc/pcabo_api.hip b/para-ortho-pca-bo_amd/csrc/pcabo_api.hip
--- a/para-ortho-pca-bo_amd/csrc/pcabo_api.hip
+++ b/para-ortho-pca-bo_amd/csrc/pcabo_api.hip
@@ -81,6 +81,7 @@
   int srv_penalty = 0;
   unsigned long long seq = 0;
   OptCrew crew;
+  double first_advance_s = 0.0;
   bool registered = false;
   bool alone = true; int alone_age = 0;
   char err[512] = {0};
@@ -855,7 +856,13 @@
   return PCABO_OK;
 }
 
-static int eval_staged(pcabo_ctx* ctx, int nq, AcqParams& p, bool allow_gemm = true) {
+struct HostWork {
+  std::function<void()> fn;
+  void run() { if (fn) { fn(); fn = nullptr; } }
+};
+static void run_beside(HostWork* w) { if (w) w->run(); }
+
+static int eval_staged(pcabo_ctx* ctx, int nq, AcqParams& p, bool allow_gemm = true, HostWork* beside = nullptr) {
   hipStream_t s = ctx->stream;
   const int k = ctx->st.k;
   const unsigned long long seq = ++ctx->seq;
@@ -883,17 +890,20 @@
   if (!small) {
     HIPCHK(hipMemcpyAsync(ctx->hVal, ctx->dVal, (size_t)nq * sizeof(double), hipMemcpyDeviceToHost, s));
     if (p.want_grad) HIPCHK(hipMemcpyAsync(ctx->hGrad, ctx->dGrad, (size_t)nq * k * sizeof(double), hipMemcpyDeviceToHost, s));
+    run_beside(beside);
     HIPCHK(wait_stream(s));
     HIPCHK(hipGetLastError());
     return PCABO_OK;
   }
+  run_beside(beside);
   return acq_published(ctx, wait_flags(ctx->hm, 0, nq, seq, deadline_in(20), &s));
 }
 
-static int score_tail(pcabo_ctx* ctx, int nq, AcqParams& p) {
+static int score_tail(pcabo_ctx* ctx, int nq, AcqParams& p, HostWork* beside = nullptr) {
   hipStream_t s = ctx->stream;
   launch_score_tail(s, nq, gp_model(ctx), p, ctx->dKS, ctx->dPartial, ctx->dVal);
   HIPCHK(hipMemcpyAsync(ctx->hVal, ctx->dVal, (size_t)nq * sizeof(double), hipMemcpyDeviceToHost, s));
+  run_beside(beside);
   HIPCHK(wait_stream(s));
   HIPCHK(hipGetLastError());
   return PCABO_OK;
@@ -928,6 +938,13 @@
   return ctx->opt_group_acq && want_grad && q <= PCABO_INLAUNCH_MAXQ && acq_group_possible(ctx->st.NP, ctx->st.k);
 }
 
+static int values_staged(pcabo_ctx* ctx, const double* Xq, int q, double best_f, int maximize, int acq, HostWork* beside = nullptr) {
+  HIPCHK(hipSetDevice(ctx->device));
+  memcpy(ctx->hXq, Xq, (size_t)q * ctx->st.k * sizeof(double));
+  AcqParams p = make_params(ctx, best_f, maximize, acq, 0);
+  return eval_staged(ctx, q, p, true, beside);
+}
+
 int pcabo_acq_eval(pcabo_ctx* ctx, const double* Xq, int q, double best_f, int maximize, int acq, double* val,
                    double* grad) {
   if (!ctx) return PCABO_ERR_ARG;
@@ -935,6 +952,11 @@
     return set_err(ctx, PCABO_ERR_ARG, "pcabo_acq_eval: bad argument or q beyond context capacity%s", "");
   if (const char* why = acq_arg_error(acq, best_f)) return set_err(ctx, PCABO_ERR_ARG, "pcabo_acq_eval: %s", why);
   if (!ctx->st.conditioned()) return set_err(ctx, PCABO_ERR_ARG, "pcabo_acq_eval: call pcabo_gp_condition first%s", "");
+  if (!grad && ctx->ptr_mode == PCABO_PTR_HOST) {
+    const int rc = values_staged(ctx, Xq, q, best_f, maximize, acq);
+    if (rc == PCABO_OK) memcpy(val, ctx->hVal, (size_t)q * sizeof(double));
+    return rc;
+  }
   HIPCHK(hipSetDevice(ctx->device));
   hipStream_t s = ctx->stream;
   const int k = ctx->st.k;
@@ -966,18 +988,12 @@
   return PCABO_OK;
 }
 
-int pcabo_gp_condition_end_eval(pcabo_ctx* ctx, const double* Xq, int q, double best_f, int maximize, int acq,
-                                double* val) {
-  if (!ctx) return PCABO_ERR_ARG;
-  if (!Xq || !val || q < 1 || q > ctx->max_q)
-    return set_err(ctx, PCABO_ERR_ARG, "pcabo_gp_condition_end_eval: bad argument or q beyond context capacity%s", "");
-  if (const char* why = acq_arg_error(acq, best_f)) return set_err(ctx, PCABO_ERR_ARG, "pcabo_gp_condition_end_eval: %s", why);
-  if (!ctx->st.in_flight()) return set_err(ctx, PCABO_ERR_ARG, "pcabo_gp_condition_end_eval: no conditioning in flight%s", "");
+static int end_eval_staged(pcabo_ctx* ctx, const double* Xq, int q, double best_f, int maximize, int acq, HostWork* beside = nullptr) {
   if (const int rc = collect_pending_wpca(ctx)) return rc;
-  if (q <= PCABO_INLAUNCH_MAXQ || ctx->ptr_mode != PCABO_PTR_HOST) {
-    int rc = pcabo_gp_condition_end(ctx);
-    if (rc != PCABO_OK) return rc;
-    return pcabo_acq_eval(ctx, Xq, q, best_f, maximize, acq, val, nullptr);
+  if (q <= PCABO_INLAUNCH_MAXQ) {
+    run_beside(beside);
+    const int rc = pcabo_gp_condition_end(ctx);
+    return rc != PCABO_OK ? rc : values_staged(ctx, Xq, q, best_f, maximize, acq);
   }
   HIPCHK(hipSetDevice(ctx->device));
   memcpy(ctx->hXq, Xq, (size_t)q * ctx->st.k * sizeof(double));
@@ -990,9 +1006,9 @@
     launch_score_ks_only(ctx->stream2, ctx->dXq, q, gp_model(ctx), p, ctx->dKS);
     HIPCHK(hipEventRecord(ctx->evKS, ctx->stream2));
     HIPCHK(hipStreamWaitEvent(ctx->stream, ctx->evKS, 0));
-    rc = score_tail(ctx, q, p);
+    rc = score_tail(ctx, q, p, beside);
   } else {
-    rc = eval_staged(ctx, q, p);
+    rc = eval_staged(ctx, q, p, true, beside);
   }
   if (rc != PCABO_OK) { ctx->st.condition_failed(); return rc; }
   if (ctx->hm->chol_info != 0) {
@@ -1003,8 +1019,25 @@
   } else {
     ctx->st.condition_ended_ok(0.0);
   }
-  memcpy(val, ctx->hVal, (size_t)q * sizeof(double));
-  return PCABO_OK;
+  return PCABO_OK;
+}
+
+int pcabo_gp_condition_end_eval(pcabo_ctx* ctx, const double* Xq, int q, double best_f, int maximize, int acq,
+                                double* val) {
+  if (!ctx) return PCABO_ERR_ARG;
+  if (!Xq || !val || q < 1 || q > ctx->max_q)
+    return set_err(ctx, PCABO_ERR_ARG, "pcabo_gp_condition_end_eval: bad argument or q beyond context capacity%s", "");
+  if (const char* why = acq_arg_error(acq, best_f)) return set_err(ctx, PCABO_ERR_ARG, "pcabo_gp_condition_end_eval: %s", why);
+  if (!ctx->st.in_flight()) return set_err(ctx, PCABO_ERR_ARG, "pcabo_gp_condition_end_eval: no conditioning in flight%s", "");
+  if (ctx->ptr_mode != PCABO_PTR_HOST) {
+    if (const int rc = collect_pending_wpca(ctx)) return rc;
+    int rc = pcabo_gp_condition_end(ctx);
+    if (rc != PCABO_OK) return rc;
+    return pcabo_acq_eval(ctx, Xq, q, best_f, maximize, acq, val, nullptr);
+  }
+  const int rc = end_eval_staged(ctx, Xq, q, best_f, maximize, acq);
+  if (rc == PCABO_OK) memcpy(val, ctx->hVal, (size_t)q * sizeof(double));
+  return rc;
 }
 
 int pcabo_logei(pcabo_ctx* ctx, const double* Xq, int q, double best_f, int maximize, double* val, double* grad) {
@@ -1081,6 +1114,9 @@
   ~ResidentSession() { stop(); }
 };
 
+static int optimize_checked(pcabo_ctx* ctx, const double* ics, int num_restarts, int batch_limit, const double* bounds, int maxiter,
+                            double best_f, int maximize, int acq, double* cand, double* vals, int* info, int* failed);
+
 int pcabo_optimize_acqf(pcabo_ctx* ctx, const double* ics, int num_restarts, int batch_limit, const double* bounds,
                         int maxiter, double best_f, int maximize, int acq, double* cand, double* vals, int* info,
                         int* failed) {
@@ -1089,6 +1125,11 @@
     return set_err(ctx, PCABO_ERR_ARG, "pcabo_optimize_acqf: bad argument%s", "");
   if (const char* why = acq_arg_error(acq, best_f)) return set_err(ctx, PCABO_ERR_ARG, "pcabo_optimize_acqf: %s", why);
   if (!ctx->st.conditioned()) return set_err(ctx, PCABO_ERR_ARG, "pcabo_optimize_acqf: call pcabo_gp_condition first%s", "");
+  return optimize_checked(ctx, ics, num_restarts, batch_limit, bounds, maxiter, best_f, maximize, acq, cand, vals, info, failed);
+}
+
+static int optimize_checked(pcabo_ctx* ctx, const double* ics, int num_restarts, int batch_limit, const double* bounds, int maxiter,
+                            double best_f, int maximize, int acq, double* cand, double* vals, int* info, int* failed) {
   HIPCHK(hipSetDevice(ctx->device));
   const int k = ctx->st.k;
   RunRestarts run;
@@ -1102,7 +1143,13 @@
   CrewCall crew(ctx->crew, run, pending);
   ResidentSession srv{ctx, p};
   for (unsigned round_no = 1;; ++round_no) {
-    crew.advance_all();
+    if (round_no == 1) {
+      const auto t = std::chrono::steady_clock::now();
+      crew.advance_all();
+      ctx->first_advance_s = std::chrono::duration<double>(std::chrono::steady_clock::now() - t).count();
+    } else {
+      crew.advance_all();
+    }
     const int nq = pack_active(run, qoff);
     if (nq == 0) break;
     int rc;
@@ -1139,6 +1186,65 @@
   if (failed) *failed = any_failed;
   return PCABO_OK;
 }
+
+int pcabo_propose_acqf(pcabo_ctx* ctx, const double* raw, int n_raw, void* blob, double eta, int num_restarts, int batch_limit,
+                       const double* bounds, int maxiter, double best_f, int maximize, int acq, int flags, double* raw_vals,
+                       int64_t* ic_idx, double* ics, double* cand, double* vals, int* info, int* failed, int* picked,
+                       double* phase_seconds) {
+  using clk = std::chrono::steady_clock;
+  if (!ctx) return PCABO_ERR_ARG;
+  if (!raw || !raw_vals || n_raw < 1 || n_raw > ctx->max_q)
+    return set_err(ctx, PCABO_ERR_ARG, "pcabo_propose_acqf: bad argument or q beyond context capacity%s", "");
+  if (!blob || !ic_idx || !ics || !picked || !bounds || !cand || !vals || num_restarts < 1 || batch_limit < 1 ||
+      num_restarts > ctx->max_q || (flags & ~PCABO_PROPOSE_NO_WAKE))
+    return set_err(ctx, PCABO_ERR_ARG, "pcabo_propose_acqf: bad argument%s", "");
+  if (n_raw < 2 || num_restarts >= n_raw)
+    return set_err(ctx, PCABO_ERR_ARG, "pcabo_propose_acqf: the pick takes fewer restarts than raw samples, of at least two%s", "");
+  if (const char* why = acq_arg_error(acq, best_f)) return set_err(ctx, PCABO_ERR_ARG, "pcabo_propose_acqf: %s", why);
+  if (acq == PCABO_ACQ_PI)
+    return set_err(ctx, PCABO_ERR_ARG, "pcabo_propose_acqf: the pick of PCABO_ACQ_PI (botorch's non-negative variant) is the caller's%s", "");
+  if (!torch_blob_ok(blob))
+    return set_err(ctx, PCABO_ERR_ARG, "pcabo_propose_acqf: not a state blob of torch's CPU generator%s", "");
+  if (ctx->ptr_mode != PCABO_PTR_HOST) return set_err(ctx, PCABO_ERR_ARG, "pcabo_propose_acqf: host pointers only%s", "");
+  const bool pending = ctx->st.in_flight();
+  if (!pending && !ctx->st.conditioned())
+    return set_err(ctx, PCABO_ERR_ARG, "pcabo_propose_acqf: call pcabo_gp_condition first%s", "");
+  *picked = 0;
+  const auto t0 = clk::now();
+  const auto since = [](clk::time_point a) { return std::chrono::duration<double>(clk::now() - a).count(); };
+  double clocks[3] = {0.0, 0.0, 0.0};
+  const auto hand_clocks = [&] { if (phase_seconds) std::copy(clocks, clocks + 3, phase_seconds); };
+  std::unique_ptr<OptCrew::Awake> awake;
+  if (!(flags & PCABO_PROPOSE_NO_WAKE) && num_restarts > batch_limit) awake.reset(new OptCrew::Awake(ctx->crew));
+  AheadPick ahead(n_raw, num_restarts);
+  HostWork draw{[&] { ahead.draw(blob); }};
+  int rc = pending ? end_eval_staged(ctx, raw, n_raw, best_f, maximize, acq, &draw)
+                   : values_staged(ctx, raw, n_raw, best_f, maximize, acq, &draw);
+  if (rc != PCABO_OK) {
+    ahead.put_back();
+    return rc;
+  }
+  draw.run();
+  memcpy(raw_vals, ctx->hVal, (size_t)n_raw * sizeof(double));
+  clocks[0] = since(t0);
+  const auto t1 = clk::now();
+  if (ahead.pick(raw_vals, eta, ic_idx) != 0) {
+    clocks[1] = since(t1);
+    hand_clocks();
+    return PCABO_OK;
+  }
+  const int k = ctx->st.k;
+  for (int j = 0; j < num_restarts; ++j) memcpy(ics + (size_t)j * k, raw + (size_t)ic_idx[j] * k, (size_t)k * sizeof(double));
+  *picked = 1;
+  clocks[1] = since(t1);
+  const auto t2 = clk::now();
+  rc = optimize_checked(ctx, ics, num_restarts, batch_limit, bounds, maxiter, best_f, maximize, acq, cand, vals, info, failed);
+  clocks[2] = since(t2);
+  hand_clocks();
+  return rc;
+}
+
+double pcabo_debug_first_advance_seconds(pcabo_ctx* ctx) { return ctx ? ctx->first_advance_s : -1.0; }
 
 int pcabo_inverse_map(pcabo_ctx* ctx, const double* z, double* x) {
   if (!ctx || !z || !x) return PCABO_ERR_ARG;
diff --git a/para-ortho-pca-bo_amd/pcabo/_native.py b/para-ortho-pca-bo_amd/pcabo/_native.py
--- a/para-ortho-pca-bo_amd/pcabo/_native.py
+++ b/para-ortho-pca-bo_amd/pcabo/_native.py
@@ -15,6 +15,8 @@
 OPT_HIDDEN_TAIL = 5
 POST_OBS_NOISE = 1
 EXTEND_BELIEVER = 1
+PROPOSE_NO_WAKE = 1
+TORCH_BLOB_BYTES = 5056
 POST_CENTRED = 2
 POST_MAX_SAMPLES = 1024
 FIT_THETA0 = (0.006737946999085467, 0.0, 0.0)
@@ -46,7 +48,7 @@
     "pcabo_acq_bounds",
     "pcabo_acq_eval", "pcabo_logei", "pcabo_gp_posterior", "pcabo_batch_gp_posterior", "pcabo_gp_posterior_sample", "pcabo_batch_gp_posterior_sample", "pcabo_gp_loo", "pcabo_batch_gp_loo",
     "pcabo_gp_extend", "pcabo_gp_truncate", "pcabo_gp_extended",
-    "pcabo_batch_gp_extend", "pcabo_batch_gp_truncate", "pcabo_batch_gp_extended", "pcabo_optimize_acqf", "pcabo_inverse_map", "pcabo_get_gp_state",
+    "pcabo_batch_gp_extend", "pcabo_batch_gp_truncate", "pcabo_batch_gp_extended", "pcabo_optimize_acqf", "pcabo_propose_acqf", "pcabo_inverse_map", "pcabo_get_gp_state",
     "pcabo_get_gram", "pcabo_lbfgsb_minimize", "pcabo_lbfgsb_set_vector_kernels", "pcabo_lbfgsb_set_sum_order", "pcabo_sobol_scramble", "pcabo_sobol_draw", "pcabo_sobol_draw_rows", "pcabo_torch_randint2", "pcabo_torch_multinomial_rows", "pcabo_boltzmann_pick_rows", "pcabo_set_profiling",
     "pcabo_get_profile", "pcabo_get_profile_calibration", "pcabo_reset_profile",
     "pcabo_batch_create", "pcabo_batch_destroy", "pcabo_batch_last_error", "pcabo_batch_ctx",
@@ -121,6 +123,8 @@
     lib.pcabo_batch_gp_extended.argtypes = [vp, ip, ip]
     lib.pcabo_optimize_acqf.argtypes = [vp, vp, C.c_int, C.c_int, vp, C.c_int, C.c_double, C.c_int, C.c_int,
                                         vp, vp, vp, ip]
+    lib.pcabo_propose_acqf.argtypes = [vp, vp, C.c_int, vp, C.c_double, C.c_int, C.c_int, vp, C.c_int, C.c_double, C.c_int, C.c_int,
+                                       C.c_int, vp, vp, vp, vp, vp, vp, ip, ip, vp]
     lib.pcabo_inverse_map.argtypes = [vp, vp, vp]
     lib.pcabo_get_gp_state.argtypes = [vp, vp, vp, vp, vp, vp]
     lib.pcabo_get_gram.argtypes = [vp, vp]
@@ -492,6 +496,31 @@
                                           _ptr(info), C.byref(failed)))
         return cand, vals, info, bool(failed.value)
 
+    def propose_acqf(self, raw, blob, num_restarts, bounds, best_f, maximize=False, acq=ACQ_LOG_EI, batch_limit=5, maxiter=200,
+                     eta=1.0, wake=True) -> dict:
+        raw = _f64(raw).reshape(-1, self.k)
+        n_raw, nr = raw.shape[0], int(num_restarts)
+        if not (isinstance(blob, np.ndarray) and blob.dtype == np.uint8 and blob.ndim == 1 and blob.size == TORCH_BLOB_BYTES
+                and blob.flags.c_contiguous and blob.flags.writeable):
+            raise ValueError(f"blob: a writable contiguous uint8 array of {TORCH_BLOB_BYTES} bytes")
+        bounds = _f64(bounds, (2, self.k))
+        raw_vals, idx = np.empty(n_raw), np.empty(max(nr, 0), dtype=np.int64)
+        ics, cand, vals = np.empty((max(nr, 0), self.k)), np.empty((max(nr, 0), self.k)), np.empty(max(nr, 0))
+        ng = (nr + batch_limit - 1) // batch_limit if nr > 0 and batch_limit > 0 else 0
+        info = np.zeros((ng, 4), dtype=np.int32)
+        failed, picked = C.c_int(0), C.c_int(0)
+        clocks = np.zeros(3)
+        rc = LIB.pcabo_propose_acqf(self._h, _ptr(raw), n_raw, _ptr(blob), float(eta), nr, int(batch_limit), _ptr(bounds),
+                                    int(maxiter), float(best_f), int(bool(maximize)), int(acq), 0 if wake else PROPOSE_NO_WAKE,
+                                    _ptr(raw_vals), _ptr(idx), _ptr(ics), _ptr(cand), _ptr(vals), _ptr(info), C.byref(failed),
+                                    C.byref(picked), _ptr(clocks))
+        self._chk(rc)
+        self._keep = None
+        out = {"raw_vals": raw_vals, "picked": bool(picked.value), "phase_seconds": clocks}
+        if picked.value:
+            out.update(ic_idx=idx, ics=ics, cand=cand, vals=vals, info=info, failed=bool(failed.value))
+        return out
+
     def inverse_map(self, z) -> np.ndarray:
         z = _f64(z).reshape(-1)
         x = np.empty(self.d)
diff --git a/para-ortho-pca-bo_amd/pcabo/acqopt.py b/para-ortho-pca-bo_amd/pcabo/acqopt.py
--- a/para-ortho-pca-bo_amd/pcabo/acqopt.py
+++ b/para-ortho-pca-bo_amd/pcabo/acqopt.py
@@ -1,5 +1,6 @@
 from __future__ import annotations
 
+import os
 import warnings
 from time import perf_counter
 from typing import Optional
@@ -70,10 +71,25 @@
     return max(s, v) if maximize else min(s, v)
 
 
+ONE_CALL_ENV = "PCABO_ONE_CALL"
+ONE_CALL_WAKE_ENV = "PCABO_ONE_CALL_WAKE"
+
+
+def one_call_default() -> bool:
+    return os.environ.get(ONE_CALL_ENV, "1") != "0"
+
+
+def one_call_applies(ctx, acq_code: int, num_restarts: int, n_raw: int) -> bool:
+    if acq_code == _native.ACQ_PI or num_restarts >= n_raw or not callable(getattr(ctx, "propose_acqf", None)):
+        return False
+    from . import hostrng
+    return hostrng.native_ok()
+
+
 def optimize_acqf(ctx: "_native.Context", bounds: np.ndarray, best_f: float, maximize: bool, acq_code: int,
                   num_restarts: int, raw_samples: int, batch_limit: int = 5, maxiter: int = 200, engine=None,
                   breakdown: Optional[dict] = None, trace: Optional[dict] = None, raw: Optional[np.ndarray] = None,
-                  raw_vals: Optional[np.ndarray] = None, before_lbfgsb=None):
+                  raw_vals: Optional[np.ndarray] = None, before_lbfgsb=None, one_call: Optional[bool] = None):
     pb = breakdown if breakdown is not None else {}
     engines = [engine] if engine is not None and raw is None else []
     ready = [raw] if raw is not None else []
@@ -97,13 +113,41 @@
             trace.update(raw_vals=vals.copy(), ic_idx=np.asarray(idx).copy())
         return raw[idx]
 
-    ics = initial_conditions()
-    if before_lbfgsb is not None:
-        before_lbfgsb()
-    t_opt = perf_counter()
-    cand, vals, info, failed = ctx.optimize_acqf(ics, bounds, best_f, maximize, acq_code, batch_limit=batch_limit,
-                                                 maxiter=maxiter)
-    pb["lbfgsb"] = pb.get("lbfgsb", 0.0) + perf_counter() - t_opt
+    def in_one_call():
+        import torch
+        blob = torch.get_rng_state().numpy()
+        if before_lbfgsb is not None:
+            before_lbfgsb()
+        r = ctx.propose_acqf(raw, blob, num_restarts, bounds, best_f, maximize, acq_code, batch_limit=batch_limit,
+                             maxiter=maxiter, eta=_init.INIT_ETA, wake=os.environ.get(ONE_CALL_WAKE_ENV, "1") != "0")
+        for key, t in zip(("raw_eval", "init_pick", "lbfgsb"), r["phase_seconds"]):
+            pb[key] = pb.get(key, 0.0) + float(t)
+        pb.setdefault("sobol", 0.0)
+        if not r["picked"]:
+            ready_vals.append(r["raw_vals"])
+            return None
+        ready.pop()
+        torch.set_rng_state(torch.from_numpy(blob))
+        if trace is not None:
+            trace.update(raw_vals=r["raw_vals"].copy(), ic_idx=r["ic_idx"].copy())
+        return r["ics"], r["cand"], r["vals"], r["info"], r["failed"]
+
+    if one_call is None:
+        one_call = one_call_default()
+    first = None
+    if one_call and raw is not None and raw_vals is None and one_call_applies(ctx, acq_code, num_restarts, len(raw)):
+        first = in_one_call()
+        before_lbfgsb = None
+    if first is not None:
+        ics, cand, vals, info, failed = first
+    else:
+        ics = initial_conditions()
+        if before_lbfgsb is not None:
+            before_lbfgsb()
+        t_opt = perf_counter()
+        cand, vals, info, failed = ctx.optimize_acqf(ics, bounds, best_f, maximize, acq_code, batch_limit=batch_limit,
+                                                     maxiter=maxiter)
+        pb["lbfgsb"] = pb.get("lbfgsb", 0.0) + perf_counter() - t_opt
     if failed:
         warnings.warn("Optimization failed in `gen_candidates_scipy`; trying again with a new set of "
                       "initial conditions.", RuntimeWarning)
@@ -122,7 +166,7 @@
 def propose(ctx: "_native.Context", bounds: np.ndarray, best_f: float, maximize: bool, acq_code: int, num_restarts: int,
             raw_samples: int, batch_limit: int = 5, maxiter: int = 200, q_eff: int = 1, strategy: str = "kriging_believer",
             f_evals=None, breakdown: Optional[dict] = None, trace: Optional[dict] = None, raw: Optional[np.ndarray] = None,
-            raw_vals: Optional[np.ndarray] = None, before_lbfgsb=None):
+            raw_vals: Optional[np.ndarray] = None, before_lbfgsb=None, one_call: Optional[bool] = None):
     believer = strategy == "kriging_believer"
     if strategy not in Q_STRATEGIES:
         raise ValueError(f"q_strategy must be one of {', '.join(Q_STRATEGIES)}; got {strategy!r}")
@@ -130,7 +174,8 @@
     s, n0, cands, infos = best_f, None, [], []
     try:
         z, _, _, info = optimize_acqf(ctx, bounds, s, maximize, acq_code, num_restarts, raw_samples, batch_limit, maxiter,
-                                      breakdown=breakdown, trace=trace, raw=raw, raw_vals=raw_vals, before_lbfgsb=before_lbfgsb)
+                                      breakdown=breakdown, trace=trace, raw=raw, raw_vals=raw_vals, before_lbfgsb=before_lbfgsb,
+                                      one_call=one_call)
         cands.append(z)
         infos.append(info)
         for _ in range(1, q_eff):
```

Result: faster. 420.0 BO iterations/s (median of 6 runs) (+4.8%).
